# eckertzhang/Text2NeRF

Hardware: AMD Instinct MI355X
Metric: ray-samples/s (render) + iters/s (train), 300^3 VM-split, 800x800 (higher is better)
Workload: dtype f32 (basis/MLP products as f16x2-split MFMA, fp32 accumulate); 1 GPU; C2 300^3 800x800 view/GPU, N=518, S1-soft seed 0, white_bg, weights=0, tile marcher; evaluated_samples_per_frame=77423712, appearance_samples_per_frame=4284741, rays_per_gpu=640000, samples_per_ray=518, warmup_frames=231, inregion_timing=none, parallelism=ray-tile x1

## Files before the change

### include/t2n.h

```cpp
#ifndef T2N_H_
#define T2N_H_

#include <stddef.h>
#include <stdint.h>

#ifdef __cplusplus
extern "C" {
#endif

typedef struct t2n_field t2n_field;
typedef void* t2n_stream;

enum {
    T2N_OK = 0,
    T2N_ERR_INVALID = -1,
    T2N_ERR_UNSUPPORTED = -2,
    T2N_ERR_HIP = -3,
    T2N_ERR_WORKSPACE = -4,
    T2N_ERR_STATE = -5
};

enum { T2N_SHADE_MLP_FEA_NOVIEW = 0, T2N_SHADE_SH = 1, T2N_SHADE_RGB = 2,
       T2N_SHADE_MLP_FEA = 3, T2N_SHADE_MLP_PE = 4, T2N_SHADE_MLP = 5 };
enum { T2N_ACT_SOFTPLUS = 0, T2N_ACT_RELU = 1 };
// ... 37 lines not shown
    const float* app_plane[3];
    const float* app_line[3];
    const float* basis_weight;
    const float* mlp_w0; const float* mlp_b0;
    const float* mlp_w1; const float* mlp_b1;
    const float* mlp_w2; const float* mlp_b2;
} t2n_field_params;

typedef struct t2n_field_grads {
    float* density_plane[3];
    float* density_line[3];
    float* app_plane[3];
    float* app_line[3];
    float* basis_weight;
    float* mlp_w0; float* mlp_b0;
    float* mlp_w1; float* mlp_b1;
    float* mlp_w2; float* mlp_b2;
} t2n_field_grads;

enum { T2N_STAT_EVALUATED = 0,
       T2N_STAT_APPEARANCE = 1,
       T2N_STAT_RAYS = 2,
       T2N_STAT_OVERFLOW = 3,
       T2N_STAT_F16_REDO = 4,
       T2N_STAT_LIST_RETRY = 5,
       T2N_STAT_COUNT = 8 };

const char* t2n_last_error(void);
int t2n_version(void);

int t2n_field_create(const t2n_field_desc* desc, t2n_field** out);
int t2n_field_destroy(t2n_field* f);
int t2n_field_upload(t2n_field* f, const t2n_field_params* p, t2n_stream stream);
int t2n_field_set_desc(t2n_field* f, const t2n_field_desc* desc);
int t2n_field_set_factor_storage(t2n_field* f, int bf16);

int t2n_field_set_mlp_precision(t2n_field* f, int exact_fp32);
int t2n_field_set_alpha_mask(t2n_field* f, const float* volume, int D, int H, int W, const float* aabb_min_host,
                             const float* inv_size_host, t2n_stream stream);
int t2n_alpha_at(const t2n_field* f, const float* xyz_world, int64_t n, float* alpha, t2n_stream stream);
int t2n_field_set_early_termination(t2n_field* f, float eps);
int t2n_field_set_feature_staging(t2n_field* f, int on);
int t2n_field_feature_staging_counts(const t2n_field* f, uint64_t out[2]);
int t2n_field_set_density_cache(t2n_field* f, int on);
int t2n_field_set_density_cache_cap(t2n_field* f, uint64_t bytes);
int t2n_field_release_density_cache(t2n_field* f);
int t2n_field_density_cache_counts(const t2n_field* f, uint64_t out[4]);
int t2n_field_density_sum_table(const t2n_field* f, const int* shift, float* out, t2n_stream stream);
#define T2N_APP_VOLUME_MIN_FRAMES 33
int t2n_field_set_appearance_volume(t2n_field* f, int on, int min_frames);
int t2n_field_set_appearance_volume_cap(t2n_field* f, uint64_t bytes);
int t2n_field_release_appearance_volume(t2n_field* f);
int t2n_field_appearance_volume_counts(const t2n_field* f, uint64_t out[4]);
int t2n_field_feature_rows(t2n_field* f, const float* app_pos, const uint32_t* counters, uint32_t list_cap, int volume, float* feat,
                           uint32_t feat_rows, t2n_stream stream);
int t2n_field_set_feature_stage_shape(t2n_field* f, int workgroups, int defer_cap);
int t2n_field_set_frame_width(t2n_field* f, int width);

int t2n_ray_directions(int H, int W, float fx, float fy, float cx, float cy, int normalize, float* dirs ,
                       t2n_stream stream);
int t2n_get_rays(const float* dirs , int64_t n, const float* c2w_host ,
                 float* rays_o , float* rays_d , float* rays6 ,
                 t2n_stream stream);
int t2n_generate_rays(int H, int W, float fx, float fy, float cx, float cy, const float* c2w_host, float* rays6,
                      t2n_stream stream);

int t2n_sample_ray(const t2n_field* f, const float* rays_o, const float* rays_d, int64_t n, int n_samples, const float* jitter, int ndc,
                   float* pts , float* z_vals , uint8_t* valid , t2n_stream stream);

int t2n_filter_rays_bbox(const t2n_field* f, const float* rays, int64_t n_rays, int ray_stride, uint8_t* mask,
                         t2n_stream stream);

int t2n_density_at(const t2n_field* f, const float* xyz_norm, int64_t n, float* feat, float* sigma, t2n_stream stream);
size_t t2n_shade_workspace_bytes(int64_t n);
int t2n_shade_at(const t2n_field* f, const float* xyz_norm, const float* viewdirs, int64_t n, float* app_feat, float* rgb,
                 void* workspace, size_t workspace_bytes, t2n_stream stream);
int t2n_raw2alpha(const float* sigma, const float* dist, int64_t n_rays, int n_samples, float* alpha, float* weights,
                  float* bg, t2n_stream stream);

size_t t2n_render_workspace_bytes(int64_t rays_per_launch, int n_samples);
size_t t2n_render_head_scratch_bytes(const t2n_field* f, int64_t n_rays);
int t2n_field_set_head_scratch_rows(t2n_field* f, int rows_per_ray);
size_t t2n_render_workspace_bytes_hint(const t2n_field* f, int64_t n_rays, int n_samples);
size_t t2n_render_workspace_bytes_budget(int64_t n_rays, int n_samples, int entries_per_ray);
uint64_t t2n_field_list_retries(const t2n_field* f);
int t2n_render_forward(t2n_field* f, const float* rays, int64_t n_rays, int ray_stride, int n_samples, uint32_t flags,
                       const float* jitter, float* rgb, float* depth, float* weights, float* z_vals, uint64_t* stats,
                       void* workspace, size_t workspace_bytes, t2n_stream stream);

typedef struct t2n_generic_desc {
    float aabb_min[3], aabb_max[3], inv_aabb_size[3];
    int32_t grid[3];
    int32_t density_n_comp[3], app_n_comp[3];
    int32_t app_dim, shading, fea_pe, view_pe, feature_c, act;
    float density_shift, distance_scale, weight_thres, step_size, near, far, z_gate;
    const float* alpha_volume;
    int32_t alpha_dims[3];
    float alpha_aabb_min[3], alpha_aabb_max[3];
} t2n_generic_desc;
size_t t2n_generic_workspace_bytes(int64_t n_rays, int n_samples);
size_t t2n_generic_workspace_bytes_desc(const t2n_generic_desc* desc, int64_t n_rays, int n_samples);
int t2n_generic_forward(const t2n_generic_desc* desc, const t2n_field_params* params, const float* rays, int64_t n_rays, int ray_stride,
                        int n_samples, uint32_t flags, const float* jitter, float* rgb, float* depth, float* weights, float* z_vals,
                        uint64_t* stats, void* workspace, size_t workspace_bytes, t2n_stream stream);
int t2n_generic_backward(const t2n_generic_desc* desc, const t2n_field_params* params, const float* rays, int64_t n_rays, int ray_stride,
                         int n_samples, uint32_t flags, const float* jitter, const float* weights, const float* z_vals,
// ... 240 lines not shown
```

### text2nerf_amd/_lib.py

```python
from __future__ import annotations

import ctypes as C
import os
import threading

_HERE = os.path.dirname(os.path.abspath(__file__))
LIB_PATH = os.environ.get("T2N_LIB") or os.path.join(_HERE, "libt2n_hip.so")

T2N_STAT_COUNT = 8
T2N_K_COUNT = 14
KERNEL_NAMES = ("march", "shade", "composite", "upload", "bwd_march", "bwd_mlp", "bwd_scatter", "density", "app_features",
                "bwd_wgrad", "bwd_density", "tv_seed", "adam", "head_step")
STAT_EVALUATED, STAT_APPEARANCE, STAT_RAYS, STAT_OVERFLOW, STAT_F16_REDO, STAT_LIST_RETRY = 0, 1, 2, 3, 4, 5

FLAG_TRAIN, FLAG_ADD_BG, FLAG_KEEP_CTX, FLAG_COHERENT, FLAG_NDC = 1, 2, 4, 8, 16
FLAG_DEVICE_ROWS = 32
FLAG_PIPELINE = 64
FLAG_GATHER_BATCH = 128
FLAG_REG_L1, FLAG_REG_ORTHO = 256, 512
REG_SLOTS = 64
SHADE_IDS = {"MLP_Fea_noview": 0, "SH": 1, "RGB": 2, "MLP_Fea": 3, "MLP_PE": 4, "MLP": 5}
ACT_IDS = {"softplus": 0, "relu": 1}
DEPTH_KINDS = {"mse": 0, "gnll": 1, "si_log": 2, "ssi": 3}
MASK_U8, MASK_I32, MASK_I64, MASK_F32, MASK_F64 = 0, 1, 2, 3, 4
# ... 32 lines not shown
                ("alpha_aabb_max", C.c_float * 3)]


class GenericBwdPlan(C.Structure):
    _fields_ = [("kernel_form", C.c_int), ("pass_rows", C.c_uint32), ("max_passes", C.c_uint32), ("workspace_bytes", C.c_size_t)]


TRAIN_HYPER_FLOATS = 32
TRAIN_HEAD_GRAD_FLOATS = 27 * 144 + 128 * 351 + 128 + 128 * 128 + 128 + 3 * 128 + 3 + 1
TRAIN_HEAD_SIZES = (27 * 144, 128 * 351, 128, 128 * 128, 128, 3 * 128, 3)


class TrainStepArgs(C.Structure):
    _fields_ = [("rays", C.c_void_p), ("n_rays", C.c_int64), ("ray_stride", C.c_int32), ("n_samples", C.c_int32),
                ("flags", C.c_uint32), ("phases", C.c_uint32),
                ("jitter", C.c_void_p), ("rgb_target", C.c_void_p), ("depth_target", C.c_void_p),
                ("w_depth", C.c_float), ("w_trans", C.c_float), ("delta", C.c_float),
                ("beta1", C.c_float), ("beta2", C.c_float), ("eps", C.c_float),
                ("hyper", C.c_void_p), ("params", FieldParams),
                ("exp_avg", C.c_void_p * 19), ("exp_avg_sq", C.c_void_p * 19),
                ("head_grads", C.c_void_p), ("rows_capacity", C.c_int64),
                ("workspace", C.c_void_p), ("workspace_bytes", C.c_size_t), ("losses", C.c_void_p), ("host_batch", C.c_void_p), ("host_batch_bytes", C.c_size_t), ("batch_buffer", C.c_void_p),
                ("shard_world", C.c_int32), ("shard_rank", C.c_int32)]


class TrainSource(C.Structure):
    _fields_ = [("rays", C.c_void_p), ("ray_stride", C.c_int32), ("rgb", C.c_void_p), ("depth", C.c_void_p), ("n_rows", C.c_int64),
                ("ids", C.c_void_p)]


_lib = None
_lock = threading.Lock()

SIGNATURES = {
    "t2n_last_error": (C.c_char_p, []),
    "t2n_version": (C.c_int, []),
    "t2n_field_create": (C.c_int, [C.POINTER(FieldDesc), C.POINTER(C.c_void_p)]),
    "t2n_field_destroy": (C.c_int, [C.c_void_p]),
    "t2n_field_upload": (C.c_int, [C.c_void_p, C.POINTER(FieldParams), C.c_void_p]),
    "t2n_field_set_desc": (C.c_int, [C.c_void_p, C.POINTER(FieldDesc)]),
    "t2n_field_set_mlp_precision": (C.c_int, [C.c_void_p, C.c_int]),
    "t2n_field_set_early_termination": (C.c_int, [C.c_void_p, C.c_float]),
    "t2n_field_set_feature_staging": (C.c_int, [C.c_void_p, C.c_int]),
    "t2n_field_feature_staging_counts": (C.c_int, [C.c_void_p, C.POINTER(C.c_uint64)]),
    "t2n_field_set_feature_stage_shape": (C.c_int, [C.c_void_p, C.c_int, C.c_int]),
    "t2n_field_set_density_cache": (C.c_int, [C.c_void_p, C.c_int]),
    "t2n_field_set_density_cache_cap": (C.c_int, [C.c_void_p, C.c_uint64]),
    "t2n_field_release_density_cache": (C.c_int, [C.c_void_p]),
    "t2n_field_density_cache_counts": (C.c_int, [C.c_void_p, C.POINTER(C.c_uint64)]),
    "t2n_field_set_appearance_volume": (C.c_int, [C.c_void_p, C.c_int, C.c_int]),
    "t2n_field_set_appearance_volume_cap": (C.c_int, [C.c_void_p, C.c_uint64]),
    "t2n_field_release_appearance_volume": (C.c_int, [C.c_void_p]),
    "t2n_field_appearance_volume_counts": (C.c_int, [C.c_void_p, C.POINTER(C.c_uint64)]),
    "t2n_field_feature_rows": (C.c_int, [C.c_void_p, C.c_void_p, C.c_void_p, C.c_uint32, C.c_int, C.c_void_p, C.c_uint32, C.c_void_p]),
    "t2n_field_density_sum_table": (C.c_int, [C.c_void_p, C.POINTER(C.c_int), C.c_void_p, C.c_void_p]),
    "t2n_sample_ray": (C.c_int, [C.c_void_p, C.c_void_p, C.c_void_p, C.c_int64, C.c_int, C.c_void_p, C.c_int, C.c_void_p, C.c_void_p,
                                 C.c_void_p, C.c_void_p]),
    "t2n_field_set_frame_width": (C.c_int, [C.c_void_p, C.c_int]),
    "t2n_field_set_alpha_mask": (C.c_int, [C.c_void_p, C.c_void_p, C.c_int, C.c_int, C.c_int, C.POINTER(C.c_float),
                                           C.POINTER(C.c_float), C.c_void_p]),
    "t2n_alpha_at": (C.c_int, [C.c_void_p, C.c_void_p, C.c_int64, C.c_void_p, C.c_void_p]),
    "t2n_ray_directions": (C.c_int, [C.c_int, C.c_int, C.c_float, C.c_float, C.c_float, C.c_float, C.c_int,
                                     C.c_void_p, C.c_void_p]),
    "t2n_get_rays": (C.c_int, [C.c_void_p, C.c_int64, C.POINTER(C.c_float), C.c_void_p, C.c_void_p, C.c_void_p,
                               C.c_void_p]),
    "t2n_generate_rays": (C.c_int, [C.c_int, C.c_int, C.c_float, C.c_float, C.c_float, C.c_float,
                                    C.POINTER(C.c_float), C.c_void_p, C.c_void_p]),
    "t2n_filter_rays_bbox": (C.c_int, [C.c_void_p, C.c_void_p, C.c_int64, C.c_int, C.c_void_p, C.c_void_p]),
    "t2n_density_at": (C.c_int, [C.c_void_p, C.c_void_p, C.c_int64, C.c_void_p, C.c_void_p, C.c_void_p]),
    "t2n_shade_workspace_bytes": (C.c_size_t, [C.c_int64]),
    "t2n_shade_at": (C.c_int, [C.c_void_p, C.c_void_p, C.c_void_p, C.c_int64, C.c_void_p, C.c_void_p, C.c_void_p,
                               C.c_size_t, C.c_void_p]),
    "t2n_raw2alpha": (C.c_int, [C.c_void_p, C.c_void_p, C.c_int64, C.c_int, C.c_void_p, C.c_void_p, C.c_void_p,
                                C.c_void_p]),
    "t2n_render_workspace_bytes": (C.c_size_t, [C.c_int64, C.c_int]),
    "t2n_render_head_scratch_bytes": (C.c_size_t, [C.c_void_p, C.c_int64]),
    "t2n_field_set_head_scratch_rows": (C.c_int, [C.c_void_p, C.c_int]),
    "t2n_render_workspace_bytes_hint": (C.c_size_t, [C.c_void_p, C.c_int64, C.c_int]),
    "t2n_field_list_retries": (C.c_uint64, [C.c_void_p]),
    "t2n_render_workspace_bytes_budget": (C.c_size_t, [C.c_int64, C.c_int, C.c_int]),
    "t2n_render_forward": (C.c_int, [C.c_void_p, C.c_void_p, C.c_int64, C.c_int, C.c_int, C.c_uint32, C.c_void_p,
                                     C.c_void_p, C.c_void_p, C.c_void_p, C.c_void_p, C.c_void_p, C.c_void_p,
                                     C.c_size_t, C.c_void_p]),
    "t2n_render_workspace_bytes_ctx": (C.c_size_t, [C.c_int64, C.c_int]),
    "t2n_depth_align_global": (C.c_int, [C.c_void_p, C.c_void_p, C.c_int, C.c_int, C.c_void_p, C.c_int, C.c_double, C.c_void_p, C.c_void_p,
                                         C.c_void_p]),
    "t2n_depth_align_fallback": (C.c_int, [C.c_void_p, C.c_void_p, C.c_int, C.c_int, C.c_double, C.c_void_p, C.c_void_p, C.c_void_p]),
    "t2n_filled_pixels_workspace_bytes": (C.c_size_t, [C.c_int, C.c_int]),
    "t2n_filled_pixels_count": (C.c_int, [C.c_void_p, C.c_int, C.c_int, C.c_void_p, C.c_void_p, C.c_void_p]),
    "t2n_filled_pixels_select": (C.c_int, [C.c_void_p, C.c_int, C.c_int, C.c_void_p, C.c_void_p, C.c_int, C.c_void_p, C.c_void_p]),
    "t2n_depth_merge_inputs": (C.c_int, [C.c_void_p, C.c_void_p, C.c_void_p, C.c_int, C.c_int, C.c_double, C.c_void_p, C.c_void_p,
                                         C.c_void_p, C.c_void_p]),
    "t2n_view_finish": (C.c_int, [C.c_void_p, C.c_void_p, C.c_void_p, C.c_int, C.c_int, C.c_double, C.c_void_p, C.c_void_p, C.c_void_p,
                                  C.c_void_p]),
    "t2n_mask_expand": (C.c_int, [C.c_void_p, C.c_int, C.c_int, C.c_void_p, C.c_void_p, C.c_void_p]),
    "t2n_mc_workspace_bytes": (C.c_size_t, [C.c_int, C.c_int, C.c_int]),
    "t2n_mc_count": (C.c_int, [C.c_void_p, C.c_int, C.c_int, C.c_int, C.c_float, C.c_void_p, C.c_void_p, C.c_void_p]),
    "t2n_mc_emit": (C.c_int, [C.c_void_p, C.c_int, C.c_int, C.c_int, C.c_float, C.c_void_p, C.POINTER(C.c_float), C.POINTER(C.c_float),
                              C.c_int, C.c_void_p, C.c_void_p, C.c_void_p, C.c_void_p]),
    "t2n_mesh_components_workspace_bytes": (C.c_size_t, [C.c_int64, C.c_int64]),
    "t2n_mesh_components": (C.c_int, [C.c_void_p, C.c_int64, C.c_int64, C.c_void_p, C.c_void_p, C.c_void_p, C.c_size_t, C.c_void_p]),
    "t2n_mesh_component_sizes": (C.c_int, [C.c_void_p, C.c_int64, C.c_void_p, C.c_int64, C.c_int64, C.c_void_p, C.c_void_p, C.c_void_p]),
    "t2n_mesh_filter_count": (C.c_int, [C.c_void_p, C.c_int64, C.c_void_p, C.c_int64, C.c_void_p, C.c_int64, C.c_void_p, C.c_size_t,
                                        C.c_void_p, C.c_void_p]),
    "t2n_mesh_filter_emit": (C.c_int, [C.c_void_p, C.c_int64, C.c_void_p, C.c_int64, C.c_void_p, C.c_int64, C.c_void_p, C.c_void_p,
                                       C.c_void_p, C.c_void_p, C.c_size_t, C.c_void_p, C.c_void_p, C.c_void_p, C.c_void_p, C.c_void_p]),
# ... 159 lines not shown
```

### text2nerf_amd/build.py

```python
from __future__ import annotations

import concurrent.futures
import glob
import os
import subprocess
import sys

HERE = os.path.dirname(os.path.abspath(__file__))
ROOT = os.path.dirname(HERE)
CSRC = os.path.join(HERE, "csrc")
LIB = os.path.join(HERE, "libt2n_hip.so")
OBJ = os.path.join(ROOT, "build", "obj")

CFLAGS = ["--offload-arch=gfx950", "-O3", "-std=c++17", "-fPIC", "-ffp-contract=off", "-fno-fast-math",
          "-munsafe-fp-atomics", "-Wall", "-Wno-unused-function", "-DNDEBUG"]
LDFLAGS = ["--offload-arch=gfx950", "-shared", "-fPIC",
           "-Wl,--no-undefined"]
FLAGS = CFLAGS + LDFLAGS[1:]
PER_FILE = {"t2n_mlp_bwd_ss.hip": ["-fno-slp-vectorize"]}


def sources():
    return sorted(glob.glob(os.path.join(CSRC, "*.hip")))


def _headers():
    return glob.glob(os.path.join(CSRC, "*.h")) + [os.path.join(ROOT, "include", "t2n.h"), __file__]


def _obj(src):
    return os.path.join(OBJ, os.path.basename(src)[:-4] + ".o")


def _stale(src):
    o = _obj(src)
    if not os.path.exists(o):
        return True
    t = os.path.getmtime(o)
    return os.path.getmtime(src) > t or any(os.path.getmtime(h) > t for h in _headers())


def needs_build():
    if not os.path.exists(LIB):
        return True
    t = os.path.getmtime(LIB)
    return any(os.path.getmtime(d) > t for d in sources() + _headers())


def check_ss3_isa(hipcc, verbose=False, extra=(), obj_dir=None):
    import re
    obj_dir = obj_dir or OBJ
    src = os.path.join(CSRC, "t2n_mlp_ss.hip")
    asm = os.path.join(obj_dir, "t2n_mlp_ss.s")
    subprocess.run([hipcc] + CFLAGS + list(extra) + ["-S", "--cuda-device-only", src, "-o", asm], check=True,
                   stderr=subprocess.DEVNULL)
    text = open(asm).read()
    found = 0
    for m in re.finditer(r"^(_ZN3t2n2ss9k_mlp_ss3\w*):[^\n]*\n(.*?)\n\.Lfunc_end\d+:", text, re.S | re.M):
        name, body = m.group(1), m.group(2)
        found += 1
        bad = [l.strip() for l in body.split("\n") if re.match(r"\s*v_accvgpr_(write|mov)", l)]
        meta = re.search(r"\.name:\s+" + name + r"\n.*?\.vgpr_spill_count:\s+(\d+)", text, re.S)
        priv = re.search(r"\.name:\s+" + name + r"\n.*?\.private_segment_fixed_size:\s+(\d+)", text, re.S)
        spills = int(meta.group(1)) if meta else -1
        scratch = int(priv.group(1)) if priv else -1
        if bad or spills != 0 or scratch != 0:
            raise RuntimeError(f"{name}: the compiler touched the AccVGPRs or spilled ({len(bad)} v_accvgpr_write/mov, {spills} spilled "
                               f"registers, {scratch} B of scratch): the hand-allocated accumulators are not safe with this build")
        if verbose:
            print(f"check_ss3_isa: {name} ok ({body.count('v_accvgpr_read_b32')} accumulator reads, no writes, no spills)", flush=True)
    if found != 2:
        raise RuntimeError(f"check_ss3_isa: expected the two instantiations of k_mlp_ss3 in the assembly, found {found}")


def build(force=False, verbose=False):
    if not force and not needs_build():
        return LIB
    hipcc = os.environ.get("HIPCC", "/opt/rocm/bin/hipcc")
    os.makedirs(OBJ, exist_ok=True)
    todo = [s for s in sources() if force or _stale(s)]

    def compile_one(src):
        cmd = [hipcc] + CFLAGS + PER_FILE.get(os.path.basename(src), []) + ["-c", src, "-o", _obj(src)]
        if verbose:
            print(" ".join(cmd), flush=True)
        subprocess.run(cmd, check=True)

    with concurrent.futures.ThreadPoolExecutor(max_workers=min(8, max(1, len(todo)))) as ex:
        list(ex.map(compile_one, todo))
    ss_obj = _obj(os.path.join(CSRC, "t2n_mlp_ss.hip"))
    stamp = ss_obj[:-2] + ".checked"
    if not os.path.exists(stamp) or os.path.getmtime(stamp) < os.path.getmtime(ss_obj):
        try:
            check_ss3_isa(hipcc, verbose)
        except Exception:
            for f in (ss_obj, stamp):
                if os.path.exists(f):
                    os.remove(f)
            raise
        open(stamp, "w").close()
    keep = {_obj(s) for s in sources()}
    for o in glob.glob(os.path.join(OBJ, "*.o")):
        if o not in keep:
            os.remove(o)
    cmd = [hipcc] + LDFLAGS + sorted(keep) + ["-o", LIB + ".tmp"]
    if verbose:
        print(" ".join(cmd), flush=True)
    subprocess.run(cmd, check=True)
    os.replace(LIB + ".tmp", LIB)
    return LIB


if __name__ == "__main__":
    if "--check-ss3" in sys.argv:
        i = sys.argv.index("--check-ss3")
        check_ss3_isa(os.environ.get("HIPCC", "/opt/rocm/bin/hipcc"), True, extra=sys.argv[i + 2:], obj_dir=sys.argv[i + 1])
        sys.exit(0)
    print(build(force="--force" in sys.argv, verbose=True))
```

### text2nerf_amd/csrc/t2n_api.hip

```cpp
#include <stdarg.h>

#include "t2n_device.h"

namespace t2n {

static thread_local char g_err[512] = "";

void set_error(const char* fmt, ...) {
    va_list ap;
    va_start(ap, fmt);
    vsnprintf(g_err, sizeof(g_err), fmt, ap);
    va_end(ap);
}

int hip_fail(hipError_t e, const char* what) {
    set_error("HIP error %d (%s) in %s", (int)e, hipGetErrorString(e), what);
    return T2N_ERR_HIP;
}

void timing_begin(t2n_field* f, int k, hipStream_t s) {
    if (!((f->timing >> k) & 1)) return;
    TimingSlot& t = f->slots[k];
    if (t.used >= kTimingEvents) return;
    if (!t.start[t.used]) {
// ... 277 lines not shown
    if (deg < 3) return;
    o[9] = (-0.5900435899266435f * y) * (3.f * xx - yy);
    o[10] = (2.890611442640554f * xy) * z;
    o[11] = (-0.4570457994644658f * y) * ((4.f * zz - xx) - yy);
    o[12] = (0.3731763325901154f * z) * ((2.f * zz - 3.f * xx) - 3.f * yy);
    o[13] = (-0.4570457994644658f * x) * ((4.f * zz - xx) - yy);
    o[14] = (1.445305721320277f * z) * (xx - yy);
    o[15] = (-0.5900435899266435f * x) * (xx - 3.f * yy);
    if (deg < 4) return;
    o[16] = (2.5033429417967046f * xy) * (xx - yy);
    o[17] = (-1.7701307697799304f * yz) * (3.f * xx - yy);
    o[18] = (0.9461746957575601f * xy) * (7.f * zz - 1.f);
    o[19] = (-0.6690465435572892f * yz) * (7.f * zz - 3.f);
    o[20] = 0.10578554691520431f * (zz * (35.f * zz - 30.f) + 3.f);
    o[21] = (-0.6690465435572892f * xz) * (7.f * zz - 3.f);
    o[22] = (0.47308734787878004f * (xx - yy)) * (7.f * zz - 1.f);
    o[23] = (-1.7701307697799304f * xz) * (xx - 3.f * yy);
    o[24] = 0.6258357354491761f * (xx * (xx - 3.f * yy) - yy * (3.f * xx - yy));
}

__global__ __launch_bounds__(256) void k_ndc_rays(int H, int W, float focal, float near, float sign, const float* __restrict__ ro,
                                                  const float* __restrict__ rd, long long n, float* o_out, float* d_out) {
    const long long i = (long long)blockIdx.x * blockDim.x + threadIdx.x;
    if (i >= n) return;
    float ox = ro[i * 3], oy = ro[i * 3 + 1], oz = ro[i * 3 + 2];
    const float dx = rd[i * 3], dy = rd[i * 3 + 1], dz = rd[i * 3 + 2];
    const float t = sign < 0.f ? -(near + oz) / dz : (near - oz) / dz;
    ox = ox + t * dx; oy = oy + t * dy; oz = oz + t * dz;
    const float kx = sign * 1.f / ((float)W / (2.f * focal)), ky = sign * 1.f / ((float)H / (2.f * focal));
    const float o0 = kx * ox / oz, o1 = ky * oy / oz;
    const float o2 = sign < 0.f ? 1.f + 2.f * near / oz : 1.f - 2.f * near / oz;
    const float d0 = kx * (dx / dz - ox / oz), d1 = ky * (dy / dz - oy / oz);
    const float d2 = sign < 0.f ? -2.f * near / oz : 2.f * near / oz;
    o_out[i * 3] = o0; o_out[i * 3 + 1] = o1; o_out[i * 3 + 2] = o2;
    d_out[i * 3] = d0; d_out[i * 3 + 1] = d1; d_out[i * 3 + 2] = d2;
}

static size_t align_up(size_t x, size_t a) { return (x + a - 1) / a * a; }

Carve carve_workspace(int64_t rays, int n_samples, bool ctx, bool feat, unsigned budget) {
    Carve c;
    c.list_cap = list_capacity_budget(rays, n_samples, budget);
    const size_t cap = (size_t)c.list_cap * kLists;
    size_t o = 0;
    c.counters = o; o = align_up(o + (size_t)kLists * kCounterStride * 4, 256);
    c.acc = o; o = align_up(o + (size_t)rays * 4, 256);
    c.ray_app = o; o = align_up(o + (size_t)rays * 16, 256);
    c.app_pos = o; o = align_up(o + cap * 16, 256);
    c.app_rgb = o; o = align_up(o + cap * 16, 256);
    c.app_ray = o; o = align_up(o + cap * 4, 256);
    c.sigma = o; if (ctx) o = align_up(o + (size_t)rays * n_samples * 4, 256);
    c.rgb_raw = o; if (ctx) o = align_up(o + (size_t)rays * 16, 256);
    c.scratch = o; if (ctx) o = align_up(o + (size_t)rays * (size_t)(n_samples / 4 > 0 ? n_samples / 4 : 1) * 16 + 256 + (size_t)rays * 4, 256);
    const size_t worst_rows = cap + (size_t)kLists * 32, want_rows = (size_t)rays * (budget && budget < 64 ? (budget + 1) / 2 : 32) + 1024;
    c.feat_rows = (unsigned)(((worst_rows < want_rows ? worst_rows : want_rows) + 127) / 128 * 128);
    if (!feat) c.feat_rows = 0;
    c.feat = o; o = align_up(o + (size_t)c.feat_rows * 32 * sizeof(float), 256);
    c.total = o;
    return c;
}
static Carve carve(int64_t rays, int n_samples) { return carve_workspace(rays, n_samples, true); }
constexpr unsigned kBudgetMin = 16;
constexpr unsigned kBudgetFloor = 2;
constexpr int64_t kBudgetMinRays = 65536;

}

using namespace t2n;

extern "C" const char* t2n_last_error(void) { return g_err; }
extern "C" int t2n_version(void) { return 100; }

extern "C" int t2n_field_create(const t2n_field_desc* desc, t2n_field** out) {
    if (!desc || !out) { set_error("t2n_field_create: NULL argument"); return T2N_ERR_INVALID; }
    t2n_field* f = new t2n_field();
    memset(&f->dev, 0, sizeof(f->dev));
    for (int k = 0; k < T2N_K_COUNT; ++k) { memset(f->slots[k].start, 0, sizeof(f->slots[k].start)); memset(f->slots[k].stop, 0, sizeof(f->slots[k].stop)); }
    const int rc = apply_desc(f, desc);
    if (rc) { delete f; return rc; }
    *out = f;
    return T2N_OK;
}

extern "C" int t2n_field_set_desc(t2n_field* f, const t2n_field_desc* d) {
    if (!f || !d) { set_error("t2n_field_set_desc: NULL argument"); return T2N_ERR_INVALID; }
    if (f->uploaded && (d->grid[0] != f->desc.grid[0] || d->grid[1] != f->desc.grid[1] || d->grid[2] != f->desc.grid[2] ||
                        d->density_n_comp != f->desc.density_n_comp || d->app_n_comp != f->desc.app_n_comp)) {
        set_error("t2n_field_set_desc: grid/n_comp change needs a new field handle");
        return T2N_ERR_STATE;
    }
    return apply_desc(f, d);
}

extern "C" int t2n_field_destroy(t2n_field* f) {
    if (!f) return T2N_OK;
    for (int k = 0; k < 3; ++k) {
        if (f->buf_den_plane[k]) (void)hipFree(f->buf_den_plane[k]);
        if (f->buf_den_line[k]) (void)hipFree(f->buf_den_line[k]);
        if (f->buf_app_plane[k]) (void)hipFree(f->buf_app_plane[k]);
        if (f->buf_app_line[k]) (void)hipFree(f->buf_app_line[k]);
        if (f->hbuf_den_plane[k]) (void)hipFree(f->hbuf_den_plane[k]);
        if (f->hbuf_den_line[k]) (void)hipFree(f->hbuf_den_line[k]);
        if (f->hbuf_app_plane[k]) (void)hipFree(f->hbuf_app_plane[k]);
        if (f->hbuf_app_line[k]) (void)hipFree(f->hbuf_app_line[k]);
    }
    if (f->gbuf_all && !f->gbuf_external) (void)hipFree(f->gbuf_all);
    if (f->buf_mlp) (void)hipFree(f->buf_mlp);
// ... 267 lines not shown
        if (carve_workspace(n_rays, n_samples, true, false).total > workspace_bytes || (uint64_t)list_capacity(n_rays, n_samples) * kLists > 0x7fffffffull) {
            set_error("t2n_render_forward: KEEP_CTX needs the whole call in one launch (workspace %zu B < %zu B)", workspace_bytes,
                      carve_workspace(n_rays, n_samples, true, false).total);
            return T2N_ERR_WORKSPACE;
        }
        if (!weights || !z_vals) { set_error("t2n_render_forward: KEEP_CTX needs weights and z_vals materialised"); return T2N_ERR_INVALID; }
    }
    int64_t per = n_rays;
    unsigned budget = 0;
    counts_poll(f, false);
    const bool generic_head = head_is_generic(f->desc.shading);
    if (tiles && !generic_head && carve(n_rays, n_samples).total > workspace_bytes && n_rays >= kBudgetMinRays && !getenv("T2N_NO_BUDGET")) {
        unsigned lo = 0, hi = (unsigned)n_samples;
        if (carve_workspace(n_rays, n_samples, true, true, kBudgetFloor).total <= workspace_bytes) {
            lo = kBudgetFloor;
            while (hi - lo > 1) {
                const unsigned mid = lo + (hi - lo) / 2;
                if (carve_workspace(n_rays, n_samples, true, true, mid).total <= workspace_bytes) lo = mid; else hi = mid;
            }
        }
        if (lo >= kBudgetFloor && (uint64_t)list_capacity_budget(n_rays, n_samples, lo) * kLists <= 0x7fffffffull) budget = lo;
    }

    const size_t head_row_bytes = generic_head ? (size_t)(32 + head_dims(f->desc).K0pad + 128 + 128) * sizeof(float) : 0;
    auto head_bytes = [&](int64_t rays) { return generic_head ? ((size_t)rays * (size_t)f->head_rows_per_ray + 32 * kLists) / 32 * 32 * head_row_bytes + 256 : (size_t)0; };
    if (!budget) {
        while (!keep && per > 1 && carve(per, n_samples).total + head_bytes(per) > workspace_bytes) per = (per + 1) / 2;
        if (!keep && carve(per, n_samples).total + head_bytes(per) > workspace_bytes) { set_error("t2n_render_forward: workspace %zu B too small", workspace_bytes); return T2N_ERR_WORKSPACE; }
        while ((uint64_t)list_capacity(per, n_samples) * kLists > 0x7fffffffull) per = (per + 1) / 2;
        if (tiles && per < n_rays) {
            const int64_t band = (int64_t)8 * f->frame_w;
            per = per / band * band;
            if (per <= 0) { set_error("t2n_render_forward: workspace too small for one 8-row band"); return T2N_ERR_WORKSPACE; }
        }
    }
    if (tiles) { const int rc = density_cache_prepare(f, s); if (rc) return rc; }
    AvolScope avol_scope{f};
    if (tiles) { const int rc = appearance_volume_prepare(f, s); if (rc) return rc; }
    char* ws = (char*)workspace;
    for (int64_t off = 0; off < n_rays; off += per) {
        const int64_t cnt = (n_rays - off) < per ? (n_rays - off) : per;
        const Carve c = carve_workspace(per, n_samples, true, !keep, budget);
        RenderLaunch L;
        L.rays = rays + off * ray_stride; L.n_rays = cnt; L.ray_stride = ray_stride; L.n_samples = n_samples; L.flags = flags;
        L.jitter = (jitter && !ndc) ? jitter + off : jitter;
        L.rgb = rgb + off * 3; L.depth = depth + off;
        L.weights = weights ? weights + off * n_samples : nullptr;
        L.z_vals = z_vals ? z_vals + off * n_samples : nullptr;
        L.stats = stats;
        L.counters = (unsigned*)(ws + c.counters); L.acc = (float*)(ws + c.acc); L.ray_app = (int4*)(ws + c.ray_app);
        L.app_pos = (float4*)(ws + c.app_pos); L.app_rgb = (float4*)(ws + c.app_rgb); L.app_ray = (int*)(ws + c.app_ray);
        L.list_cap = c.list_cap;
        L.feat = (float*)(ws + c.feat); L.feat_rows = c.feat_rows;
        L.sigma_ctx = keep ? (float*)(ws + c.sigma) : nullptr;
        L.rgb_raw = keep ? (float4*)(ws + c.rgb_raw) : nullptr;
        int rc;
        const KeptRows kr = keep && f->desc.shading == T2N_SHADE_MLP_FEA_NOVIEW ? kept_rows(c.total, workspace_bytes) : KeptRows{0, 0, 0, 0, 0};
        {
            SetupOps so;
            const bool mark = kr.rows >= 32;
            if (!mark) so.zero(L.counters, (size_t)kLists * kCounterStride * 4);
            else {
                const unsigned lo = kKeptMagicWord < kKeptRowsWord ? kKeptMagicWord : kKeptRowsWord, hi = kKeptMagicWord < kKeptRowsWord ? kKeptRowsWord : kKeptMagicWord;
                so.zero(L.counters, (size_t)lo * 4);
                if (hi > lo + 1) so.zero(L.counters + lo + 1, (size_t)(hi - lo - 1) * 4);
                if ((unsigned)(kLists * kCounterStride) > hi + 1) so.zero(L.counters + hi + 1, (size_t)(kLists * kCounterStride - hi - 1) * 4);
                so.set(L.counters + kKeptMagicWord, kKeptMagic);
                so.set(L.counters + kKeptRowsWord, (unsigned)kr.rows);
            }
            if (stats_pending) { so.zero(stats, sizeof(uint64_t) * T2N_STAT_COUNT); stats_pending = false; }
            if (tiles) {
                const int cap_e = n_samples / 4 > 0 ? n_samples / 4 : 1;
                so.zero(ws + c.scratch + (size_t)cnt * cap_e * 16, 4);
            }
            if ((rc = launch_setup(so, s))) return rc;
        }
        if (tiles) {
            if ((rc = launch_march_tiles(f, L, f->frame_w, (int)(cnt / f->frame_w), (float*)(ws + c.sigma), (float4*)(ws + c.scratch), s))) return rc;
        } else if ((rc = launch_march(f, L, s))) return rc;
        if (budget) counts_post(f, L.counters, n_rays, n_samples, budget, s);
        if (keep && (rc = ctx_counts_post(workspace, L.counters, s))) return rc;
        if (generic_head) {
            const HeadDims H = head_dims(f->desc);
            HeadPlanDev* plan = (HeadPlanDev*)(L.counters + kHeadPlanWord);
            if ((rc = launch_head_plan(L.counters, L.list_cap, plan, s))) return rc;
            const size_t off = align_up(c.total, 256);
            size_t avail = workspace_bytes > off ? workspace_bytes - off : 0;
            long long cap = (long long)(avail / head_row_bytes) / 32 * 32;
            if (cap > 0x7fffffe0ll) cap = 0x7fffffe0ll;
            if (cap < 32) {
                set_error("t2n_render_forward: the workspace holds no activation row of the general head (add t2n_render_head_scratch_bytes)");
                return T2N_ERR_WORKSPACE;
            }
            {
                float* feat32 = (float*)(ws + off); float* x0 = feat32 + cap * 32; float* h0 = x0 + cap * H.K0pad; float* h1 = h0 + cap * 128;
                const long long worst = ((long long)L.list_cap + 31) / 32 * 32 * kLists;
                const long long worst_rows = worst < (cnt * (long long)n_samples + 32ll * kLists) ? worst : (cnt * (long long)n_samples + 32ll * kLists);
                for (long long row0 = 0; row0 < worst_rows; row0 += cap) {
                    ShadeCtx ctx{nullptr, feat32 - row0 * 32, nullptr, nullptr};
                    if ((rc = launch_shade_list(f, L.app_pos, L.app_ray, L.rays, ray_stride, L.counters, L.list_cap, L.app_rgb, &ctx, s, true,
                                                (unsigned)(row0 + cap), nullptr, 0, nullptr, (unsigned)(row0 / 32), (unsigned)((row0 + cap) / 32)))) return rc;
                    if ((rc = launch_head_forward(f, nullptr, cap, feat32, L.app_pos, L.app_ray, L.rays, ray_stride, L.counters, L.list_cap, x0, h0,
                                                  h1, L.app_rgb, s, plan, row0))) return rc;
                }
            }
        } else {
            if (kr.rows >= 32) {
                ShadeCtx ctx{(float*)(ws + kr.x144), (float*)(ws + kr.feat32), (float*)(ws + kr.h0), (float*)(ws + kr.h1)};
                if ((rc = launch_shade_list(f, L.app_pos, L.app_ray, L.rays, ray_stride, L.counters, L.list_cap, L.app_rgb, &ctx, s, false, kr.rows))) return rc;
            } else if ((rc = launch_shade_list(f, L.app_pos, L.app_ray, L.rays, ray_stride, L.counters, L.list_cap, L.app_rgb, nullptr, s, false,
                                               0xffffffffu, keep ? nullptr : L.feat, L.feat_rows, stats))) return rc;
        }
        if ((rc = tiles ? launch_composite(f, L, s, f->frame_w, (int)(cnt / f->frame_w)) : launch_composite(f, L, s))) return rc;
        if (tiles && finish_supported(f) && (rc = launch_finish_rays(f, L, (const float*)(ws + c.sigma), (const float4*)(ws + c.scratch), s))) return rc;
    }
    return T2N_OK;
}

extern "C" size_t t2n_render_workspace_bytes_hint(const t2n_field* f, int64_t n_rays, int n_samples) {
    if (!f || n_rays <= 0 || n_samples <= 0) return 0;
    counts_poll(const_cast<t2n_field*>(f), false);
    const size_t worst = carve(n_rays, n_samples).total;
    if (n_rays < kBudgetMinRays) return worst;
    unsigned b = f->list_hint ? 2u * f->list_hint + 16u : 32u;
    if (b < kBudgetMin) b = kBudgetMin;
    if (b >= (unsigned)n_samples) return worst;
    const size_t want = carve_workspace(n_rays, n_samples, true, true, b).total;
    return want < worst ? want : worst;
}
extern "C" uint64_t t2n_field_list_retries(const t2n_field* f) {
    if (!f) return 0;
    counts_poll(const_cast<t2n_field*>(f), true);
    return f->list_retries;
}
extern "C" size_t t2n_render_workspace_bytes_budget(int64_t n_rays, int n_samples, int entries_per_ray) {
    if (n_rays <= 0 || n_samples <= 0 || entries_per_ray < 0) return 0;
    return carve_workspace(n_rays, n_samples, true, true, (unsigned)entries_per_ray).total;
}

extern "C" int t2n_field_set_alpha_mask(t2n_field* f, const float* volume, int D, int H, int W, const float* aabb_min_host,
                                        const float* inv_size_host, t2n_stream stream) {
    if (!f) { set_error("t2n_field_set_alpha_mask: NULL field"); return T2N_ERR_INVALID; }
    if (f->buf_alpha) { T2N_HIP(hipStreamSynchronize((hipStream_t)stream)); (void)hipFree(f->buf_alpha); f->buf_alpha = nullptr; }
    f->dev.alpha = nullptr;
    if (!volume) return T2N_OK;
    if (D < 1 || H < 1 || W < 1 || !aabb_min_host || !inv_size_host) { set_error("t2n_field_set_alpha_mask: bad argument"); return T2N_ERR_INVALID; }
    const size_t bytes = (size_t)D * H * W * sizeof(float);
    T2N_HIP(hipMalloc((void**)&f->buf_alpha, bytes));
    T2N_HIP(hipMemcpyAsync(f->buf_alpha, volume, bytes, hipMemcpyDeviceToDevice, (hipStream_t)stream));
    f->dev.alpha = f->buf_alpha; f->dev.aD = D; f->dev.aH = H; f->dev.aW = W;
    for (int k = 0; k < 3; ++k) { f->dev.a_min[k] = aabb_min_host[k]; f->dev.a_inv[k] = inv_size_host[k]; }
    return T2N_OK;
}

extern "C" int t2n_field_set_head_scratch_rows(t2n_field* f, int rows_per_ray) {
    if (!f || rows_per_ray < 1 || rows_per_ray > 4096) { set_error("t2n_field_set_head_scratch_rows: rows_per_ray must lie in [1, 4096]"); return T2N_ERR_INVALID; }
    f->head_rows_per_ray = rows_per_ray;
    return T2N_OK;
}

extern "C" int t2n_field_set_frame_width(t2n_field* f, int width) {
    if (!f || width < 0) { set_error("t2n_field_set_frame_width: bad argument"); return T2N_ERR_INVALID; }
    f->frame_w = width;
    return T2N_OK;
}

extern "C" int t2n_field_set_factor_storage(t2n_field* f, int bf16) {
    if (!f) { set_error("t2n_field_set_factor_storage: NULL field"); return T2N_ERR_INVALID; }
    if ((bf16 != 0) != (f->factor_bf16 != 0)) f->uploaded = false;
    f->factor_bf16 = bf16 ? 1 : 0;
    if (!f->factor_bf16)
        for (int k = 0; k < 3; ++k) {
            f->dev.den.plane_h[k] = f->dev.den.line_h[k] = f->dev.app.plane_h[k] = f->dev.app.line_h[k] = nullptr;
        }
    return T2N_OK;
}

// ... 9 lines not shown
extern "C" int t2n_field_set_mlp_precision(t2n_field* f, int exact_fp32) {
    if (!f) { set_error("t2n_field_set_mlp_precision: NULL field"); return T2N_ERR_INVALID; }
    f->mlp_split = exact_fp32 ? 0 : 1;
    return T2N_OK;
}

extern "C" int t2n_field_set_feature_staging(t2n_field* f, int on) {
    if (!f) { set_error("t2n_field_set_feature_staging: NULL field"); return T2N_ERR_INVALID; }
    f->feature_staging = on ? 1 : 0;
    return T2N_OK;
}

extern "C" int t2n_field_set_density_cache(t2n_field* f, int on) {
    if (!f) { set_error("t2n_field_set_density_cache: NULL field"); return T2N_ERR_INVALID; }
    f->dcache_on = on ? 1 : 0;
    return T2N_OK;
}
extern "C" int t2n_field_set_density_cache_cap(t2n_field* f, uint64_t bytes) {
    if (!f) { set_error("t2n_field_set_density_cache_cap: NULL field"); return T2N_ERR_INVALID; }
    f->dcache_cap = (size_t)bytes;
    f->dcache_alloc_failed = false;
    return T2N_OK;
}
extern "C" int t2n_field_release_density_cache(t2n_field* f) {
    if (!f) { set_error("t2n_field_release_density_cache: NULL field"); return T2N_ERR_INVALID; }
    density_cache_release(f);
    return T2N_OK;
}
extern "C" int t2n_field_density_cache_counts(const t2n_field* f, uint64_t out[4]) {
    if (!f || !out) { set_error("t2n_field_density_cache_counts: NULL argument"); return T2N_ERR_INVALID; }
    out[0] = f->dcache_counts[0]; out[1] = f->dcache_counts[1]; out[2] = f->dcache_counts[2]; out[3] = (uint64_t)f->dcache_bytes;
    return T2N_OK;
}
extern "C" int t2n_field_set_appearance_volume(t2n_field* f, int on, int min_frames) {
    if (!f || min_frames < 0) { set_error("t2n_field_set_appearance_volume: NULL field or min_frames < 0"); return T2N_ERR_INVALID; }
    f->avol_on = on ? 1 : 0;
    f->avol_min_frames = min_frames ? min_frames : T2N_APP_VOLUME_MIN_FRAMES;
    return T2N_OK;
}
extern "C" int t2n_field_set_appearance_volume_cap(t2n_field* f, uint64_t bytes) {
    if (!f) { set_error("t2n_field_set_appearance_volume_cap: NULL field"); return T2N_ERR_INVALID; }
    f->avol_cap = (size_t)bytes;
    f->avol_alloc_failed = false;
    return T2N_OK;
}
extern "C" int t2n_field_release_appearance_volume(t2n_field* f) {
    if (!f) { set_error("t2n_field_release_appearance_volume: NULL field"); return T2N_ERR_INVALID; }
    appearance_volume_release(f);
    return T2N_OK;
}
extern "C" int t2n_field_appearance_volume_counts(const t2n_field* f, uint64_t out[4]) {
    if (!f || !out) { set_error("t2n_field_appearance_volume_counts: NULL argument"); return T2N_ERR_INVALID; }
    out[0] = (uint64_t)f->avol_bytes; out[1] = f->avol_counts[2]; out[2] = f->avol_counts[0]; out[3] = f->avol_counts[1];
    return T2N_OK;
}
extern "C" int t2n_field_feature_rows(t2n_field* f, const float* app_pos, const uint32_t* counters, uint32_t list_cap, int volume, float* feat,
                                      uint32_t feat_rows, t2n_stream stream) {
    if (!f || !app_pos || !counters || !feat || feat_rows % 32u) { set_error("t2n_field_feature_rows: bad argument"); return T2N_ERR_INVALID; }
    if (!f->uploaded) { set_error("t2n_field_feature_rows: the field has no uploaded parameters"); return T2N_ERR_STATE; }
    if (f->desc.shading != T2N_SHADE_MLP_FEA_NOVIEW || !f->mlp_split) { set_error("t2n_field_feature_rows: needs the fused MLP_Fea_noview head on split products"); return T2N_ERR_UNSUPPORTED; }
    hipStream_t s = (hipStream_t)stream;
    AvolScope avol_scope{f};
    f->dev.avol = nullptr;
    if (volume) {
        const int on = f->avol_on, mf = f->avol_min_frames;
        f->avol_on = 1; f->avol_min_frames = 1;
        const int rc = appearance_volume_prepare(f, s);
        f->avol_on = on; f->avol_min_frames = mf;
        if (rc) return rc;
        if (!f->dev.avol) { set_error("t2n_field_feature_rows: this field gets no feature volume (cap, addressing, allocation)"); return T2N_ERR_UNSUPPORTED; }
    }
    return launch_feature_rows(f, (const float4*)app_pos, counters, list_cap, feat, feat_rows, s);
}
extern "C" int t2n_field_density_sum_table(const t2n_field* f, const int* shift, float* out, t2n_stream stream) {
    if (!f || !shift || !out) { set_error("t2n_field_density_sum_table: NULL argument"); return T2N_ERR_INVALID; }
    if (!f->uploaded) { set_error("t2n_field_density_sum_table: the field has no uploaded factors"); return T2N_ERR_STATE; }
    return launch_density_sum_table(f, out, shift, (hipStream_t)stream);
}

extern "C" int t2n_field_set_feature_stage_shape(t2n_field* f, int workgroups, int defer_cap) {
    if (!f) { set_error("t2n_field_set_feature_stage_shape: NULL field"); return T2N_ERR_INVALID; }
    if (workgroups < 0 || defer_cap < 0 || defer_cap > 64) { set_error("t2n_field_set_feature_stage_shape: workgroups >= 0, defer_cap in [0, 64]"); return T2N_ERR_INVALID; }
    f->feature_workgroups = workgroups;
    f->feature_defer_cap = defer_cap ? defer_cap : 16;
    return T2N_OK;
}

extern "C" int t2n_field_feature_staging_counts(const t2n_field* f, uint64_t out[2]) {
    if (!f || !out) { set_error("t2n_field_feature_staging_counts: NULL argument"); return T2N_ERR_INVALID; }
    out[0] = out[1] = 0;
    if (!f->staging_counts) return T2N_OK;
    T2N_HIP(hipDeviceSynchronize());
    unsigned long long h[2];
    T2N_HIP(hipMemcpy(h, f->staging_counts, sizeof(h), hipMemcpyDeviceToHost));
    out[0] = h[0]; out[1] = h[1];
    return T2N_OK;
}

extern "C" int t2n_timing_enable(t2n_field* f, int on) {
    if (!f) return T2N_ERR_INVALID;
    f->timing = on == 0 ? 0 : (on == 1 ? (1 << T2N_K_COUNT) - 1 : (on >> 1) & ((1 << T2N_K_COUNT) - 1));
    return T2N_OK;
}

extern "C" int t2n_timing_read(t2n_field* f, double* ms, int64_t* launches, int reset) {
    if (!f || !ms || !launches) { set_error("t2n_timing_read: NULL argument"); return T2N_ERR_INVALID; }
// ... 8 lines not shown
```

### text2nerf_amd/csrc/t2n_app_volume.hip

```cpp
#include "t2n_internal.h"
#include "t2n_device.h"

namespace t2n {

constexpr int kAvK = 144;

struct AvBuildArgs { FactorSet app; const float* Bt; float* out; int n[3]; long long corners; };

template <int K>
__device__ __forceinline__ void av_pair(const AvBuildArgs& a, const float* __restrict__ Bs, const int c[3], float (&acc)[28]) {
    const float4* __restrict__ P = reinterpret_cast<const float4*>(a.app.plane[K]) + ((size_t)c[mat1(K)] * a.app.W[K] + c[mat0(K)]) * 12;
    const float4* __restrict__ L = reinterpret_cast<const float4*>(a.app.line[K]) + (size_t)c[vecm(K)] * 12;
#pragma unroll 1
    for (int q = 0; q < 12; ++q) {
        const float4 p = P[q], l = L[q];
        const float x[4] = {p.x * l.x, p.y * l.y, p.z * l.z, p.w * l.w};
        const float4* __restrict__ b = reinterpret_cast<const float4*>(Bs + (48 * K + 4 * q) * 32);
#pragma unroll
        for (int ch = 0; ch < 4; ++ch)
#pragma unroll
            for (int jq = 0; jq < 7; ++jq) {
                const float4 bv = b[ch * 8 + jq];
                acc[4 * jq] = fmaf(bv.x, x[ch], acc[4 * jq]); acc[4 * jq + 1] = fmaf(bv.y, x[ch], acc[4 * jq + 1]);
                acc[4 * jq + 2] = fmaf(bv.z, x[ch], acc[4 * jq + 2]); acc[4 * jq + 3] = fmaf(bv.w, x[ch], acc[4 * jq + 3]);
            }
    }
}

__global__ __launch_bounds__(256) void k_app_volume_build(const AvBuildArgs a) {
    __shared__ __attribute__((aligned(16))) float Bs[kAvK * 32];
    for (int i = threadIdx.x; i < kAvK * 32 / 4; i += 256) reinterpret_cast<float4*>(Bs)[i] = reinterpret_cast<const float4*>(a.Bt)[i];
    __syncthreads();
    const long long idx = (long long)blockIdx.x * 256 + threadIdx.x;
    if (idx >= a.corners) return;
    const int nx = a.n[0] + 1, ny = a.n[1] + 1;
    const int x = (int)(idx % nx), y = (int)((idx / nx) % ny), z = (int)(idx / ((long long)nx * ny));
    const int c[3] = {min(x, a.n[0] - 1), min(y, a.n[1] - 1), min(z, a.n[2] - 1)};
    float acc[28];
#pragma unroll
    for (int j = 0; j < 28; ++j) acc[j] = 0.f;
    av_pair<0>(a, Bs, c, acc);
    av_pair<1>(a, Bs, c, acc);
    av_pair<2>(a, Bs, c, acc);
    float4* __restrict__ o = reinterpret_cast<float4*>(a.out + (size_t)idx * kAvStride);
#pragma unroll
    for (int jq = 0; jq < 7; ++jq) o[jq] = make_float4(acc[4 * jq], acc[4 * jq + 1], acc[4 * jq + 2], jq == 6 ? 0.f : acc[4 * jq + 3]);
    if constexpr (kAvStride == 32) o[7] = make_float4(0.f, 0.f, 0.f, 0.f);
}

struct AvReadArgs {
    FactorSet app;
    const float* avol; unsigned row, slice, ny1;
    const float4* app_pos; const unsigned* counters; unsigned list_cap; int nlists; unsigned tile_hi;
    float* feat;
};

__global__ __launch_bounds__(256) void k_app_features_vol(const AvReadArgs a) {
    constexpr int LPE = 4, NQ = 8 / LPE, EPP = 64 / LPE, PASSES = 32 / EPP;
    const int lane = threadIdx.x & 63, wid = __builtin_amdgcn_readfirstlane((int)(threadIdx.x >> 6));
    unsigned cnt_l = 0;
    if (lane < a.nlists) {
        cnt_l = a.counters[lane * kCounterStride];
        if (cnt_l > a.list_cap) cnt_l = a.list_cap;
    }
    unsigned incl = (cnt_l + 31u) / 32u;
#pragma unroll
    for (int o = 1; o < 8; o <<= 1) {
        const unsigned t = __shfl_up(incl, o);
        if (lane >= o) incl += t;
    }
    unsigned ntiles = (unsigned)__builtin_amdgcn_readfirstlane((int)__shfl(incl, a.nlists - 1));
    if (ntiles > a.tile_hi) ntiles = a.tile_hi;
    const unsigned wave_stride = gridDim.x * 4u;
    const int e = lane / LPE, q = lane % LPE;
    const char* __restrict__ V = reinterpret_cast<const char*>(a.avol);
    for (unsigned tile = blockIdx.x * 4u + wid; tile < ntiles; tile += wave_stride) {
        const int li = (int)__popcll(__ballot((lane < a.nlists) & (incl <= tile)));
        const unsigned before = li ? __shfl(incl, li - 1) : 0u;
        const unsigned lbase = (unsigned)li * a.list_cap;
        const unsigned base = (unsigned)__builtin_amdgcn_readfirstlane((int)(lbase + (tile - before) * 32u));
        const unsigned count = lbase + __shfl(cnt_l, li);
        const unsigned nlive = (unsigned)__builtin_amdgcn_readfirstlane((int)(count - base < 32u ? count - base : 32u));
        const float4* __restrict__ pb = a.app_pos + base;
        asm volatile("" : "+s"(pb));
        float* __restrict__ rb = a.feat + (size_t)tile * 1024;
        asm volatile("" : "+s"(rb));
        float4 pos[PASSES];
#pragma unroll
        for (int p = 0; p < PASSES; ++p) pos[p] = (unsigned)(EPP * p + e) < nlive ? pb[EPP * p + e] : make_float4(0.f, 0.f, 0.f, 0.f);
#pragma unroll
        for (int p = 0; p < PASSES; ++p) {
            const bool live = (unsigned)(EPP * p + e) < nlive;
            const float4 mine = pos[p];
            const Axes3 A = sample_axes_inbox(a.app, mine.x, mine.y, mine.z);
            const unsigned ix = (unsigned)min(max(A.a[0].i0, 0), a.app.W[0] - 1), iy = (unsigned)min(max(A.a[1].i0, 0), a.app.H[0] - 1);
            const unsigned iz = (unsigned)min(max(A.a[2].i0, 0), a.app.H[1] - 1);
            const unsigned cell = umad24(umad24(iz, a.ny1, iy), a.row, ix * kAvCornerBytes);
            const unsigned o00 = (live ? cell : 0u) + (unsigned)q * 16u;
            const unsigned o01 = o00 + a.row, o10 = o00 + a.slice, o11 = o10 + a.row;
            const unsigned off[4] = {o00, o01, o10, o11};
            float4 c[4][2][NQ];
#pragma unroll
            for (int zy = 0; zy < 4; ++zy)
#pragma unroll
                for (int x = 0; x < 2; ++x)
#pragma unroll
                    for (int i = 0; i < NQ; ++i)
                        c[zy][x][i] = *reinterpret_cast<const float4*>(V + (size_t)off[zy] + ((int)kAvCornerBytes * x + 16 * LPE * i));
            __builtin_amdgcn_sched_barrier(0);
            const float wx0 = live ? A.a[0].w0 : 0.f, wx1 = live ? A.a[0].w1 : 0.f;
            const float wyx[2][2] = {{A.a[1].w0 * wx0, A.a[1].w0 * wx1}, {A.a[1].w1 * wx0, A.a[1].w1 * wx1}};
            const float wz[2] = {A.a[2].w0, A.a[2].w1};
            float4 r[NQ];
#pragma unroll
            for (int zy = 0; zy < 4; ++zy)
#pragma unroll
                for (int x = 0; x < 2; ++x) {
                    const float w = wyx[zy & 1][x] * wz[zy >> 1];
#pragma unroll
                    for (int i = 0; i < NQ; ++i) r[i] = (zy == 0 && x == 0) ? f4_mul(c[0][0][i], w) : f4_fma(c[zy][x][i], w, r[i]);
                }
            if (q == 6 % LPE) r[6 / LPE].w = live ? mine.w : 0.f;
            if (q == 7 % LPE) r[7 / LPE] = make_float4(0.f, 0.f, 0.f, 0.f);
            float* __restrict__ row = rb + (unsigned)((EPP * p + e) * 32 + 4 * q);
#pragma unroll
            for (int i = 0; i < NQ; ++i) *reinterpret_cast<float4*>(row + 4 * LPE * i) = r[i];
        }
    }
}

int launch_app_features_vol(t2n_field* f, const float4* app_pos, const unsigned* counters_dev, unsigned list_cap, unsigned tile_hi, float* feat,
                            hipStream_t s) {
    AvReadArgs a;
    a.app = f->dev.app;
    a.avol = f->dev.avol; a.row = f->dev.av_row; a.slice = f->dev.av_slice; a.ny1 = (unsigned)f->desc.grid[1] + 1u;
    a.app_pos = app_pos; a.counters = counters_dev; a.list_cap = list_cap; a.nlists = kLists; a.tile_hi = tile_hi; a.feat = feat;
    const unsigned long long wg = ((unsigned long long)tile_hi + 3u) / 4u;
    const unsigned wg_max = 256u * 8u;
    const dim3 grid((unsigned)(wg < wg_max ? (wg ? wg : 1u) : wg_max));
    hipLaunchKernelGGL(k_app_features_vol, grid, dim3(256), 0, s, a);
    T2N_HIP(hipGetLastError());
    return T2N_OK;
}

size_t appearance_volume_bytes(const t2n_field* f) {
    const int* g = f->desc.grid;
    return (size_t)(g[0] + 1) * (g[1] + 1) * (g[2] + 1) * kAvCornerBytes;
}

int launch_app_volume_build(const t2n_field* f, float* out, hipStream_t s) {
    AvBuildArgs a;
    a.app = f->dev.app; a.Bt = f->dev.basisA; a.out = out;
    a.corners = 1;
    for (int k = 0; k < 3; ++k) { a.n[k] = f->desc.grid[k]; a.corners *= a.n[k] + 1; }
    hipLaunchKernelGGL(k_app_volume_build, dim3((unsigned)((a.corners + 255) / 256)), dim3(256), 0, s, a);
    T2N_HIP(hipGetLastError());
    return T2N_OK;
}

void appearance_volume_release(t2n_field* f) {
    if (f->avol) { (void)hipDeviceSynchronize(); (void)hipFree(f->avol); }
    f->avol = nullptr; f->avol_bytes = 0; f->avol_version = 0; f->avol_seen = 0; f->avol_run = 0; f->avol_alloc_failed = false;
    f->dev.avol = nullptr;
}

int appearance_volume_prepare(t2n_field* f, hipStream_t s) {
    f->dev.avol = nullptr;
    if (f->avol_seen == f->app_version) ++f->avol_run; else { f->avol_seen = f->app_version; f->avol_run = 1; }
    const auto direct = [&]() { ++f->avol_counts[1]; return (int)T2N_OK; };
    if (!f->avol_on) return direct();
    if (f->desc.shading != T2N_SHADE_MLP_FEA_NOVIEW || !f->mlp_split || f->desc.app_n_comp != 48 || f->desc.app_dim != 27) return direct();
    const int* g = f->desc.grid;
    const size_t bytes = appearance_volume_bytes(f);
    size_t cap = f->avol_cap;
    if (!cap) {
        static size_t dev_total[64] = {};
        int d = 0;
        if (hipGetDevice(&d) != hipSuccess) { (void)hipGetLastError(); d = 0; }
        size_t& total = dev_total[(unsigned)d % 64u];
// ... 36 lines not shown
```

### text2nerf_amd/csrc/t2n_internal.h

```cpp
#pragma once
#include <hip/hip_runtime.h>
#include <stdint.h>
#include <stdio.h>
#include <string.h>

#include "../../include/t2n.h"

namespace t2n {

constexpr int kWave = 64;
constexpr int kMaxSamples = 8192;
constexpr int kAppDimMax = 32;

__host__ __device__ constexpr int mat0(int k) { return k == 2 ? 1 : 0; }
__host__ __device__ constexpr int mat1(int k) { return k == 0 ? 1 : 2; }
__host__ __device__ constexpr int vecm(int k) { return 2 - k; }

struct FactorSet {
    const float* plane[3];
    const float* line[3];
    int W[3], H[3], L[3];
    int C;
    const void* plane_h[3];
    const void* line_h[3];
// ... 57 lines not shown
    void* buf_mlp_h = nullptr;
    const unsigned* split_unsafe = nullptr;
    void* buf_ss = nullptr;
    bool ss_dirty = true;
    void* ss_event = nullptr; void* ss_stream = nullptr;
    unsigned* ss_ok_host = nullptr; void* ss_ok_event = nullptr; int ss_variant = -2;
    float* buf_alpha = nullptr;
    int mlp_split = 1;
    int feature_staging = 1;
    unsigned long long* staging_counts = nullptr;
    int feature_defer_cap = 16;
    int feature_workgroups = 0;
    float* gbuf_den_plane[3] = {nullptr, nullptr, nullptr};
    float* gbuf_den_line[3] = {nullptr, nullptr, nullptr};
    float* gbuf_app_plane[3] = {nullptr, nullptr, nullptr};
    float* gbuf_app_line[3] = {nullptr, nullptr, nullptr};
    bool gbuf_external = false;
    float* gbuf_all = nullptr; size_t gbuf_bytes = 0;
    t2n_field_params params_ref;
    bool uploaded = false;
    int timing = 0;
    int frame_w = 0;
    int head_rows_per_ray = 32;
    float term_eps = 0.f;
    t2n::TimingSlot slots[T2N_K_COUNT];
    static constexpr int kCountSlots = 4;
    struct CountSlot { unsigned* host = nullptr; void* ev = nullptr; bool pending = false; int64_t n_rays = 0; int n_samples = 0; unsigned budget = 0; };
    CountSlot count_slots[kCountSlots]; int count_next = 0;
    void* side_stream = nullptr; void* ev_fork = nullptr; void* ev_join = nullptr;
    void* ev_den = nullptr;
    unsigned* plan_host = nullptr; unsigned plan_seq = 0;
    void* ev_pack = nullptr;
    void* gemm_stream = nullptr; void* ev_fork2 = nullptr; void* ev_join2 = nullptr;
    void* train_dev = nullptr; unsigned* train_host = nullptr; void* train_ev[12] = {};
    unsigned train_calls = 0; bool train_chain = false;
    bool train_packed = false;
    t2n_train_source train_src = {}; bool train_src_set = false;
    bool train_src_fresh = false;
    unsigned list_hint = 0;
    void* reg_ws = nullptr; size_t reg_ws_bytes = 0;
    unsigned long long list_retries = 0;
    float* dcache = nullptr; size_t dcache_bytes = 0;
    unsigned long long den_version = 1, dcache_version = 0, dcache_seen = 0;
    int dcache_on = 1; size_t dcache_cap = 0;
    bool dcache_alloc_failed = false;
    void* dcache_ev = nullptr; void* dcache_stream = nullptr;
    unsigned long long dcache_counts[3] = {0, 0, 0};
    float* avol = nullptr; size_t avol_bytes = 0;
    unsigned long long app_version = 1, avol_version = 0, avol_seen = 0, avol_run = 0;
    int avol_on = 1, avol_min_frames = T2N_APP_VOLUME_MIN_FRAMES; size_t avol_cap = 0;
    bool avol_alloc_failed = false;
    void* avol_ev = nullptr; void* avol_stream = nullptr;
    unsigned long long avol_counts[3] = {0, 0, 0};
};

namespace t2n {

void set_error(const char* fmt, ...);
int hip_fail(hipError_t e, const char* what);

#define T2N_HIP(call)                                        \
    do {                                                     \
        hipError_t e__ = (call);                             \
        if (e__ != hipSuccess) return t2n::hip_fail(e__, #call); \
    } while (0)

void counts_poll(t2n_field* f, bool wait);
void timing_begin(t2n_field* f, int k, hipStream_t s);
void timing_end(t2n_field* f, int k, hipStream_t s);

int launch_relayout(t2n_field* f, const t2n_field_params* p, hipStream_t s);
int launch_pack_mlp(t2n_field* f, const t2n_field_params* p, hipStream_t s, unsigned* absmax_out = nullptr);

struct RenderLaunch {
    const float* rays; int64_t n_rays; int ray_stride; int n_samples; uint32_t flags;
    const float* jitter; float* rgb; float* depth; float* weights; float* z_vals; uint64_t* stats;
    float* acc; int4* ray_app; unsigned* counters; float4* app_pos; int* app_ray; float4* app_rgb; unsigned list_cap;
    float* feat = nullptr; unsigned feat_rows = 0;
    float* sigma_ctx; float4* rgb_raw;
};
int launch_march(t2n_field* f, const RenderLaunch& L, hipStream_t s);
int launch_ray_stats(const RenderLaunch& L, hipStream_t s);
int launch_filter_bbox(const FieldDev& F, const float* rays, long long n_rays, int ray_stride, uint8_t* mask, hipStream_t s);
int launch_filter_alpha(const FieldDev& F, const float* rays, long long n_rays, int ray_stride, int n_samples, uint8_t* mask, hipStream_t s);
size_t density_cache_bytes(const t2n_field* f);
int density_cache_prepare(t2n_field* f, hipStream_t s);
void density_cache_release(t2n_field* f);
int launch_density_sum_table(const t2n_field* f, float* out, const int shift[3], hipStream_t s);
#ifndef T2N_AVOL_STRIDE
#define T2N_AVOL_STRIDE 32
#endif
constexpr int kAvStride = T2N_AVOL_STRIDE;
constexpr int kAvFeatures = 27;
constexpr unsigned kAvCornerBytes = kAvStride * sizeof(float);
static_assert(kAvStride % 4 == 0 && kAvStride >= 28 && kAvStride <= 32, "corner stride: whole quads that hold the 27 features");
struct AvolScope { t2n_field* f; ~AvolScope() { f->dev.avol = nullptr; } };
size_t appearance_volume_bytes(const t2n_field* f);
int appearance_volume_prepare(t2n_field* f, hipStream_t s);
void appearance_volume_release(t2n_field* f);
int launch_app_volume_build(const t2n_field* f, float* out, hipStream_t s);
int launch_app_features_vol(t2n_field* f, const float4* app_pos, const unsigned* counters_dev, unsigned list_cap, unsigned tile_hi, float* feat,
                            hipStream_t s);
int launch_feature_rows(t2n_field* f, const float4* app_pos, const unsigned* counters_dev, unsigned list_cap, float* feat, unsigned feat_rows,
                        hipStream_t s);
int launch_march_tiles(t2n_field* f, const RenderLaunch& L, int img_w, int img_h, float* spill, float4* scratch, hipStream_t s);
constexpr int kLists = 8;
constexpr int kCounterStride = 64;
inline unsigned list_capacity(long long n_rays, int n_samples) {
    const unsigned nblocks = (unsigned)((n_rays + 3) / 4);
    return ((nblocks >> 3) + ((nblocks & 7u) ? 1u : 0u)) * 4u * (unsigned)n_samples + (unsigned)n_samples;
}
inline unsigned list_capacity_budget(long long n_rays, int n_samples, unsigned budget) {
    const unsigned worst = list_capacity(n_rays, n_samples);
    if (budget == 0 || budget >= (unsigned)n_samples) return worst;
    const unsigned long long per = ((unsigned long long)n_rays * budget + kLists - 1) / kLists + (unsigned)n_samples;
    return per < worst ? (unsigned)per : worst;
}
struct ShadeCtx { float* x144; float* feat32; float* h0; float* h1; };
int launch_shade_list(t2n_field* f, const float4* app_pos, const int* app_ray, const float* rays, int ray_stride,
                      const unsigned* counters_dev, unsigned list_cap, float4* app_rgb, const ShadeCtx* ctx, hipStream_t s,
                      bool features_only = false, unsigned ctx_rows = 0xffffffffu, float* feat = nullptr, unsigned feat_rows = 0,
                      uint64_t* stats = nullptr, unsigned tile_lo = 0, unsigned tile_hi = 0xffffffffu);
constexpr int kRangeFlagWord = 32;
constexpr int kKeptMagicWord = 33, kKeptRowsWord = 34;
constexpr int kOverflowWord = 35;
constexpr int kHeadPlanWord = 40;
constexpr int kFailEntriesWord = 36;
constexpr unsigned kKeptMagic = 0x4b455054u;
int launch_mlp_ss(t2n_field* f, const float* feat, const unsigned* counters_dev, unsigned list_cap, unsigned tile_hi, float4* app_rgb,
                  unsigned* range_flag, hipStream_t s);

struct HeadDims { int shading, C, fea_pe, view_pe, pos_pe, o_feat, o_view, o_pe_a, n_pe_a, o_pe_v, n_pe_v, K0, K0pad; };
HeadDims head_dims(const t2n_field_desc& d);
inline bool head_is_generic(int shading) { return shading == T2N_SHADE_MLP_FEA || shading == T2N_SHADE_MLP_PE || shading == T2N_SHADE_MLP; }
struct HeadPlanDev { unsigned t[kLists + 1]; unsigned rows; };
int launch_head_plan(const unsigned* counters, unsigned list_cap, HeadPlanDev* plan, hipStream_t s);
int launch_dense_rows(const float* IN, int ldin, const float* Wt, int K, int N, const float* bias, int relu, long long rows, float* OUT, int ldo,
                      hipStream_t s, const HeadPlanDev* plan, long long row0);
int launch_head_forward(t2n_field* f, const unsigned tiles_before[kLists + 1], long long rows, const float* feat32, const float4* app_pos,
                        const int* app_ray, const float* rays, int ray_stride, const unsigned* counters, unsigned list_cap, float* x0,
                        float* h0, float* h1, float4* app_rgb, hipStream_t s, const HeadPlanDev* plan = nullptr, long long row0 = 0);
int launch_head_in_bwd(t2n_field* f, const float* gx, const float* feat32, long long rows, float* gf, hipStream_t s);
struct SetupOps {
    unsigned* zero_ptr[6]; unsigned long long zero_words[6]; int nz = 0;
    unsigned* set_ptr[4]; unsigned set_val[4]; int ns = 0;
    bool overflow = false;
    void zero(void* p, size_t bytes) {
        if (!p || !bytes) return;
        if (nz >= 6) { overflow = true; return; }
        zero_ptr[nz] = (unsigned*)p; zero_words[nz] = (bytes + 3) / 4; ++nz;
    }
    void set(void* p, unsigned v) {
        if (ns >= 4) { overflow = true; return; }
        set_ptr[ns] = (unsigned*)p; set_val[ns] = v; ++ns;
    }
};
int launch_setup(const SetupOps& o, hipStream_t s);
int launch_simple_head_bwd(t2n_field* f, const unsigned tiles_before[kLists + 1], long long rows, const float4* go, const float4* app_rgb,
                           const int* app_ray, const float* rays, int ray_stride, const unsigned* counters, unsigned list_cap, float* gf,
                           hipStream_t s);

size_t gemm_h_pack_bytes(int K0);
int gemm_h_pack(t2n_field* f, void* buf, int K0, hipStream_t s);
int launch_gemm_nn_h(void* packbuf, int which, int K0, const float* IN, int ldin, long long rows, const float* ACT, int ldact, float* OUT,
                     int ldo, hipStream_t s);
int launch_gemm_tn_b(const float* A, int lda, const float* B, int ldb, long long rows, int N, float* part, int ldp, int chunk_rows,
                     int ng, int chunks, bool pe, float* db, hipStream_t s, const unsigned* rows_dev = nullptr);
struct TnPlan { int chunk_rows, chunks, ng, ldp; };
TnPlan tn_plan(int64_t rows, int N);
size_t tn_part_bytes(int64_t rows, int k0);
bool gemm_fp32_mode(const t2n_field* f);
void launch_bwd_l2(const float4* go, const float* h1, long long rows, const float* w2, float* g1, float* dw2, float* db2, float* scratch,
                   hipStream_t s, const unsigned* rows_dev = nullptr);
void launch_gemm_tn(int MB, bool fp32, const float* A, int lda, const float* B, int ldb, long long rows, int M, int N, float* C, int ldc,
                    float* part, hipStream_t s, const float* pe_feat = nullptr, float* db = nullptr, const unsigned* rows_dev = nullptr,
                    bool reduce = true);
struct WgradRegions { size_t l2, tn[3], total; };
WgradRegions wgrad_regions(int64_t rows, int k0);
void launch_wgrad_reduce(const char* base, long long rows, float* dw2, float* db2, float* dw1, float* dw0, float* dwb, hipStream_t s,
                         const float* loss_part = nullptr, long long n_rays = 0, float w_depth = 0.f, float w_trans = 0.f, float* losses = nullptr);
void launch_gemm_nn(const float* IN, int ldin, const float* W, int ldw, long long rows, int K, int N, const float* ACT, int ldact, float* OUT,
                    int ldo, hipStream_t s);
void launch_colsum(const float* G, int ld, long long rows, int N, float* db, hipStream_t s);
// ... 41 lines not shown
```

### text2nerf_amd/csrc/t2n_march_tiles.hip

```cpp
#include "t2n_device.h"

namespace t2n {

constexpr int kMaxLog2W = 2;
constexpr int kDStrideMax = (1 << (2 * kMaxLog2W)) + 4;
constexpr int kPairFloats = 3 * 16 * kDStrideMax;
constexpr int kSumFloats = 96;
constexpr int kStageFloats = kPairFloats + kSumFloats;
static_assert(63 + 21 < kSumFloats && kStageFloats % 4 == 0, "summed table: the farthest read stays in the wave's region; 16-B aligned regions");
typedef float f32x4_t __attribute__((ext_vector_type(4)));

struct TileArgs {
    FieldDev F;
    const float* rays; long long n_rays; int ray_stride; int n_samples; int img_w, img_h;
    float* acc; float* depth; int4* ray_app;
    float* wbuf;
    float4* scratch; int cap; unsigned* ovf_count; int* ovf_list;
    float4* app_pos; int* app_ray; unsigned* counters; unsigned list_cap; unsigned long long* stats;
    float* dense_w;
#ifdef MT_PROF
    unsigned long long* prof;
#endif
};

__device__ __forceinline__ void lds_fence_w() {
    __builtin_amdgcn_fence(__ATOMIC_RELEASE, "wavefront");
    __builtin_amdgcn_wave_barrier();
    __builtin_amdgcn_fence(__ATOMIC_ACQUIRE, "wavefront");
}

template <int CTRL>
__device__ __forceinline__ int dpp_shr(int v, int identity) {
    return __builtin_amdgcn_update_dpp(identity, v, CTRL, 0xf, 0xf, false);
}
__device__ __forceinline__ int wave_min_i(int v) {
    const int big = 0x7fffffff;
    v = min(v, dpp_shr<0x111>(v, big));
    v = min(v, dpp_shr<0x112>(v, big));
    v = min(v, dpp_shr<0x114>(v, big));
    v = min(v, dpp_shr<0x118>(v, big));
    const int a = __builtin_amdgcn_readlane(v, 15), b = __builtin_amdgcn_readlane(v, 31);
    const int c = __builtin_amdgcn_readlane(v, 47), d = __builtin_amdgcn_readlane(v, 63);
    return min(min(a, b), min(c, d));
}
__device__ __forceinline__ int wave_max_i(int v) {
    const int small = -0x7fffffff;
    v = max(v, dpp_shr<0x111>(v, small));
    v = max(v, dpp_shr<0x112>(v, small));
    v = max(v, dpp_shr<0x114>(v, small));
    v = max(v, dpp_shr<0x118>(v, small));
    const int a = __builtin_amdgcn_readlane(v, 15), b = __builtin_amdgcn_readlane(v, 31);
    const int c = __builtin_amdgcn_readlane(v, 47), d = __builtin_amdgcn_readlane(v, 63);
    return max(max(a, b), max(c, d));
}

__device__ __forceinline__ unsigned wave_or_u(unsigned v) {
    v |= (unsigned)dpp_shr<0x111>((int)v, 0);
    v |= (unsigned)dpp_shr<0x112>((int)v, 0);
    v |= (unsigned)dpp_shr<0x114>((int)v, 0);
    v |= (unsigned)dpp_shr<0x118>((int)v, 0);
    const unsigned a = (unsigned)__builtin_amdgcn_readlane((int)v, 15), b = (unsigned)__builtin_amdgcn_readlane((int)v, 31);
    const unsigned c = (unsigned)__builtin_amdgcn_readlane((int)v, 47), d = (unsigned)__builtin_amdgcn_readlane((int)v, 63);
    return (a | b) | (c | d);
}

template <int LOG2W>
__device__ __forceinline__ void table_build(const FactorSet& S, const int (&amn)[3], float* __restrict__ stD, int l15, int lq) {
    constexpr int WS = 1 << LOG2W, SL = WS * WS, NB = SL / 16, ST = SL + 4;
    const int gs[3] = {S.W[0], S.H[0], S.H[1]};
    float4 av[3][NB], bv[3];
#pragma unroll
    for (int k = 0; k < 3; ++k) {
// ... 55 lines not shown
__device__ __forceinline__ CellTaps cached_load(const FieldDev& F, unsigned off) {
    const char* __restrict__ B = reinterpret_cast<const char*>(F.dsum);
    CellTaps t;
    t.d00 = *reinterpret_cast<const F2U*>(B + off);
    t.d01 = *reinterpret_cast<const F2U*>(B + (off + F.ds_row));
    t.d10 = *reinterpret_cast<const F2U*>(B + (off + F.ds_slice));
    t.d11 = *reinterpret_cast<const F2U*>(B + (off + F.ds_slice + F.ds_row));
    return t;
}
__device__ __forceinline__ float cached_read3(const Axes3& A, const CellTaps& t) {
    const Axis& ax = A.a[0];
    const Axis& ay = A.a[1];
    const Axis& az = A.a[2];
    const float wnw = ay.w0 * ax.w0, wne = ay.w0 * ax.w1, wsw = ay.w1 * ax.w0, wse = ay.w1 * ax.w1;
    float v0 = t.d00.a * wnw, v1 = t.d10.a * wnw;
    v0 = fmaf(t.d00.b, wne, v0); v1 = fmaf(t.d10.b, wne, v1);
    v0 = fmaf(t.d01.a, wsw, v0); v1 = fmaf(t.d11.a, wsw, v1);
    v0 = fmaf(t.d01.b, wse, v0); v1 = fmaf(t.d11.b, wse, v1);
    return fmaf(v1, az.w1, v0 * az.w0);
}

template <int K>
__device__ __forceinline__ float pair_dot_global(const FactorSet& S, const Axes3& A, float part) {
    const Axis& ax = A.a[mat0(K)];
    const Axis& ay = A.a[mat1(K)];
    const Axis& al = A.a[vecm(K)];
    const float4* __restrict__ P = reinterpret_cast<const float4*>(S.plane[K]);
    const float4* __restrict__ L = reinterpret_cast<const float4*>(S.line[K]);
    const unsigned W = (unsigned)S.W[K];
    const unsigned nw = ((unsigned)ay.i0 * W + ax.i0) * 4, ne = ((unsigned)ay.i0 * W + ax.i1) * 4;
    const unsigned sw = ((unsigned)ay.i1 * W + ax.i0) * 4, se = ((unsigned)ay.i1 * W + ax.i1) * 4;
#pragma unroll 1
    for (int q = 0; q < 4; ++q) {
        float4 v = f4_mul(P[nw + q], ay.w0 * ax.w0);
        v = f4_fma(P[ne + q], ay.w0 * ax.w1, v);
        v = f4_fma(P[sw + q], ay.w1 * ax.w0, v);
        v = f4_fma(P[se + q], ay.w1 * ax.w1, v);
        float4 l = f4_mul(L[al.i0 * 4 + q], al.w0);
        l = f4_fma(L[al.i1 * 4 + q], al.w1, l);
        part = fmaf(v.x, l.x, part); part = fmaf(v.y, l.y, part); part = fmaf(v.z, l.z, part); part = fmaf(v.w, l.w, part);
    }
    return part;
}

__device__ __forceinline__ void void_entries(float4* __restrict__ app_pos, int* __restrict__ app_ray, unsigned list, unsigned list_cap,
                                             unsigned lo, unsigned hi, int lane) {
    if (hi > list_cap) hi = list_cap;
    for (unsigned e = lo + (unsigned)lane; e < hi; e += 64u) {
        app_pos[(size_t)list * list_cap + e] = make_float4(0.f, 0.f, 0.f, 0.f);
        app_ray[(size_t)list * list_cap + e] = 0;
    }
}

constexpr int kDenseLd = 20;
constexpr int kDenseFloats = 64 * kDenseLd;
struct __attribute__((aligned(4))) F4U { float x, y, z, w; };

#ifndef T2N_MT_WAVES
#define T2N_MT_WAVES 5
#endif
#ifndef T2N_MTD_WAVES
#define T2N_MTD_WAVES 4
#endif
#ifndef T2N_MTC_WAVES
#define T2N_MTC_WAVES 5
#endif
#ifndef T2N_MTCD_WAVES
#define T2N_MTCD_WAVES 4
#endif
#ifdef MT_PROF
#define MT_T(var) do { const unsigned long long tn = __builtin_readcyclecounter(); var += tn - p_t; p_t = tn; } while (0)
#else
#define MT_T(var) do {} while (0)
#endif
constexpr int mt_waves(bool dense, bool cached) { return cached ? (dense ? T2N_MTCD_WAVES : T2N_MTC_WAVES) : (dense ? T2N_MTD_WAVES : T2N_MT_WAVES); }
template <bool DENSE, bool ALPHA = false, bool RELU = false, bool CACHED = false>
__global__ __launch_bounds__(256) __attribute__((amdgpu_waves_per_eu(mt_waves(DENSE, CACHED), mt_waves(DENSE, CACHED)))) void k_march_tiles(const TileArgs a) {
    extern __shared__ __attribute__((aligned(16))) float smem[];
    const int lane = threadIdx.x & 63, wid = threadIdx.x >> 6;
    const int l15 = lane & 15, lq = lane >> 4;
    float* __restrict__ stD = smem + (size_t)wid * kStageFloats;
    if constexpr (!CACHED) {
        for (int i = lane; i < kStageFloats; i += 64) stD[i] = 0.f;
        lds_fence_w();
    }
    float* __restrict__ wt = smem + (CACHED ? 0 : 4 * kStageFloats) + (size_t)wid * kDenseFloats;
    const FieldDev& F = a.F;
    const int tiles_x = (a.img_w + 7) >> 3;
    const long long tile = (long long)blockIdx.x * 4 + wid;
    const int ty = (int)(tile / tiles_x), tx = (int)(tile - (long long)ty * tiles_x);
    const int px = tx * 8 + (lane & 7), py = ty * 8 + (lane >> 3);
    if (ty * 8 >= a.img_h) return;
    const bool have = px < a.img_w && py < a.img_h;
    const long long r = have ? (long long)py * a.img_w + px : 0;
    const int N = a.n_samples;
    Ray ray;
    if (have) ray = load_ray(F, a.rays + r * a.ray_stride, a.ray_stride);
    else { ray.ox = ray.oy = ray.oz = 1e30f; ray.dx = ray.dy = ray.dz = 0.f; ray.tmin = 0.f; ray.last = 0.f; }
    int lo = N, hi = -1;
    if (have) ray_interval<false>(F, ray, N, lo, hi);
    const int wlo = wave_min_i(lo), whi = wave_max_i(hi);

    float T = 1.f, acc = 0.f, dep = 0.f;
    int first = -1, last = -1;
    unsigned napp = 0;
    int nev = 0;
    int ovf_from = 0;

    long long frow[4];
    if constexpr (DENSE) {
#pragma unroll
        for (int j = 0; j < 4; ++j) {
            const int rho = (lane >> 2) + 16 * j;
            const int fx = tx * 8 + (rho & 7), fy = ty * 8 + (rho >> 3);
            frow[j] = (fx < a.img_w && fy < a.img_h) ? ((long long)fy * a.img_w + fx) * N : -1;
        }
    }
    constexpr int kSteps = 2;
    const int i_begin = DENSE ? (wlo & ~15) : wlo, i_end = DENSE ? min(N - 1, whi | 15) : whi;
    const float eps = DENSE ? 0.f : F.term_eps;
    bool dead = false;
#ifdef MT_PROF
    unsigned long long p_coord = 0, p_axes = 0, p_build = 0, p_read = 0, p_act = 0, p_pairs = 0;
    const unsigned long long p_start = __builtin_readcyclecounter();
    unsigned long long p_t = p_start;
#endif
    for (int i = i_begin; i <= i_end; i += kSteps) {
        if (eps > 0.f && (((i - i_begin) & 15) == 0)) {
            dead = T < eps;
// ... 136 lines not shown
            }
        }
#ifdef MT_PROF
        MT_T(p_act); ++p_pairs;
#endif
    }
#ifdef MT_PROF
    if (lane == 0 && a.prof) {
        unsigned long long* o = a.prof + (size_t)(blockIdx.x * 4 + wid) * 8;
        o[0] = p_coord; o[1] = p_axes; o[2] = p_build; o[3] = p_read; o[4] = p_act; o[5] = p_pairs; o[6] = __builtin_readcyclecounter() - p_start;
    }
#endif
    const int Lw = last >= first && first >= 0 ? last - first + 1 : 0;
    if (have) {
        a.acc[r] = acc;
        a.depth[r] = dep + (1.f - acc) * ray.last;
    }
    const bool over = have && napp > (unsigned)a.cap;
    const unsigned n = (have && !over) ? napp : 0u;
    unsigned incl = n;
#pragma unroll
    for (int o = 1; o < 64; o <<= 1) {
        const unsigned t = __shfl_up(incl, o);
        if (lane >= o) incl += t;
    }
    const unsigned total = __shfl(incl, 63);
    const unsigned list = blockIdx.x & 7u;
    unsigned base = 0;
    if (lane == 0 && total) base = atomicAdd(&a.counters[list * kCounterStride], total);
    base = __shfl(base, 0);
    const bool fits = base + total <= a.list_cap;
    if (!fits && total) void_entries(a.app_pos, a.app_ray, list, a.list_cap, base, base + total, lane);
    const unsigned slot0 = list * a.list_cap + base + (incl - n);
    if (have) {
        if (over || !fits) {
            const unsigned k = atomicAdd(a.ovf_count, 1u);
            a.ovf_list[k] = (int)r;
            a.ray_app[r] = make_int4(ovf_from, (int)napp, nev, Lw > 0 ? (first | (Lw << 11)) : 0);
        } else {
            a.ray_app[r] = make_int4((int)slot0, fits ? (int)n : 0, nev, Lw > 0 ? (first | (Lw << 11)) : 0);
            if (fits) {
                const float4* __restrict__ src = a.scratch + (size_t)r * a.cap;
                for (unsigned k = 0; k < n; k += 4) {
                    const float4 e0 = src[k], e1 = src[k + 1 < n ? k + 1 : n - 1], e2 = src[k + 2 < n ? k + 2 : n - 1],
                                 e3 = src[k + 3 < n ? k + 3 : n - 1];
                    a.app_pos[slot0 + k] = e0; a.app_ray[slot0 + k] = (int)r;
                    if (k + 1 < n) { a.app_pos[slot0 + k + 1] = e1; a.app_ray[slot0 + k + 1] = (int)r; }
                    if (k + 2 < n) { a.app_pos[slot0 + k + 2] = e2; a.app_ray[slot0 + k + 2] = (int)r; }
                    if (k + 3 < n) { a.app_pos[slot0 + k + 3] = e3; a.app_ray[slot0 + k + 3] = (int)r; }
                }
            }
        }
    }
}

struct CompactArgs {
    FieldDev F;
    const float* rays; long long n_rays; int ray_stride; int n_samples;
    const float* wbuf;
    int4* ray_app; float4* app_pos; int* app_ray; unsigned* counters; unsigned list_cap;
    unsigned long long* stats;
    const float4* scratch; int cap;
    int finisher;
};
__device__ __forceinline__ void reserve_slots(const CompactArgs& a, long long r, unsigned list, int lane, const int4 ra, unsigned& slot0,
                                              unsigned& napp, int* ovf_slot) {
    slot0 = 0;
    if (lane == 0) {
        bool fits = napp == 0;
        for (unsigned att = 0; att < (unsigned)kLists && !fits; ++att) {
            const unsigned l = (list + att) & (unsigned)(kLists - 1);
            if (a.counters[l * kCounterStride] + napp > a.list_cap) continue;
            const unsigned s0 = atomicAdd(&a.counters[l * kCounterStride], napp);
            if (s0 + napp <= a.list_cap) { slot0 = l * a.list_cap + s0; fits = true; }
            else
                for (unsigned e = s0; e < a.list_cap; ++e) {
                    a.app_pos[(size_t)l * a.list_cap + e] = make_float4(0.f, 0.f, 0.f, 0.f);
                    a.app_ray[(size_t)l * a.list_cap + e] = 0;
                }
        }
        if (fits || !a.finisher) a.ray_app[r] = make_int4((int)slot0, fits ? (int)napp : 0, ra.z, ra.w);
        else {
            a.ray_app[r] = make_int4(-ra.x - 1, (int)napp, ra.z, ra.w);
            *ovf_slot = (int)((unsigned)r | 0x80000000u);
            atomicAdd(&a.counters[kFailEntriesWord], napp);
        }
        if (!fits && !a.finisher && a.stats) a.stats[T2N_STAT_OVERFLOW] = 1ull;
        if (!fits) a.counters[kOverflowWord] = 1u;
        if (!fits) napp = 0;
    }
    slot0 = __shfl(slot0, 0);
    napp = __shfl(napp, 0);
}
__device__ __forceinline__ void compact_span(const CompactArgs& a, long long r, const Ray& ray, int from, int end, unsigned slot0, unsigned run,
                                             int lane) {
    const FieldDev& F = a.F;
    const int N = a.n_samples;
    for (int base = from; base < end; base += 64) {
        const int i = base + lane;
        const float w = i < end ? a.wbuf[r * N + i] : 0.f;
        const bool m = (i < end) & (w > F.thres);
        const unsigned long long bal = __ballot(m);
        if (m) {
            const unsigned pre = (unsigned)__popcll(bal & ((1ull << lane) - 1ull));
            const float z = sample_z<false>(F, ray, i, 0.f);
            float xn, yn, zn;
            sample_point<false>(F, ray, z, xn, yn, zn);
            const unsigned s = slot0 + run + pre;
            a.app_pos[s] = make_float4(xn, yn, zn, w);
            a.app_ray[s] = (int)r;
        }
        run += (unsigned)__popcll(bal);
    }
}
__device__ __forceinline__ void compact_ray_staged(const CompactArgs& a, long long r, unsigned list, int lane, int* ovf_slot) {
    const int4 ra = a.ray_app[r];
    const int first = ra.w & 2047, Lw = ra.w >> 11, from = ra.x;
    unsigned napp = (unsigned)ra.y, slot0;
    reserve_slots(a, r, list, lane, ra, slot0, napp, ovf_slot);
    const unsigned staged = napp < (unsigned)a.cap ? napp : (unsigned)a.cap;
    for (unsigned k = (unsigned)lane; k < staged; k += 64u) {
        a.app_pos[slot0 + k] = a.scratch[(size_t)r * a.cap + k];
        a.app_ray[slot0 + k] = (int)r;
    }
    if (napp > staged) {
        const Ray ray = load_ray(a.F, a.rays + r * a.ray_stride, a.ray_stride);
        compact_span(a, r, ray, from, first + Lw, slot0, staged, lane);
    }
}
__global__ __launch_bounds__(256) void k_compact_list(const CompactArgs a, const unsigned* ovf_count, int* ovf_list) {
    const int lane = threadIdx.x & 63;
    const unsigned n = *ovf_count;
    for (unsigned k = blockIdx.x * 4u + (threadIdx.x >> 6); k < n; k += gridDim.x * 4u)
        compact_ray_staged(a, ovf_list[k], blockIdx.x & 7u, lane, ovf_list + k);
}

__global__ __launch_bounds__(256) void k_dense_fill(const FieldDev F, const float* __restrict__ rays, long long n_rays, int ray_stride, int N,
                                                    float* __restrict__ w, float* __restrict__ z) {
    const int lane = threadIdx.x & 63;
    const long long r = (long long)blockIdx.x * 4 + (threadIdx.x >> 6);
    if (r >= n_rays) return;
    Ray ray;
    if (z) ray = load_ray(F, rays + r * ray_stride, ray_stride);
    for (int i = lane; i < N; i += 64) {
        if (z) z[r * N + i] = sample_z<false>(F, ray, i, 0.f);
        if (w) w[r * N + i] = 0.f;
    }
}

struct SumTableArgs { FactorSet den; float* out; int n[3]; int nb[3]; int shift[3]; long long boxes; };
__global__ __launch_bounds__(256) void k_density_sum_table(const SumTableArgs a) {
    __shared__ __attribute__((aligned(16))) float smem[4 * kStageFloats];
    const int lane = threadIdx.x & 63, wid = threadIdx.x >> 6;
    const long long box = (long long)blockIdx.x * 4 + wid;
    if (box >= a.boxes) return;
    float* __restrict__ stD = smem + (size_t)wid * kStageFloats;
    const int bx = (int)(box % a.nb[0]), by = (int)((box / a.nb[0]) % a.nb[1]), bz = (int)(box / ((long long)a.nb[0] * a.nb[1]));
    const int o[3] = {4 * bx - a.shift[0], 4 * by - a.shift[1], 4 * bz - a.shift[2]};
    const int amn[3] = {max(o[0], 0), max(o[1], 0), max(o[2], 0)};
    table_build<2>(a.den, amn, stD, lane & 15, lane >> 4);
    lds_fence_w();
    table_sum<2>(stD, lane);
    lds_fence_w();
    const int x = amn[0] + (lane & 3), y = amn[1] + ((lane >> 2) & 3), z = amn[2] + (lane >> 4);
    if (x < o[0] + 4 && y < o[1] + 4 && z < o[2] + 4 && x <= a.n[0] && y <= a.n[1] && z <= a.n[2])
        a.out[((size_t)z * (a.n[1] + 1) + y) * (a.n[0] + 1) + x] = stD[lane];
}

size_t density_cache_bytes(const t2n_field* f) {
    const int* g = f->desc.grid;
    return (size_t)(g[0] + 1) * (g[1] + 1) * (g[2] + 1) * sizeof(float);
}

int launch_density_sum_table(const t2n_field* f, float* out, const int shift[3], hipStream_t s) {
    SumTableArgs a;
    a.den = f->dev.den; a.out = out;
    a.boxes = 1;
    for (int k = 0; k < 3; ++k) {
        if (shift[k] < 0 || shift[k] > 3) { set_error("density sum table: shift[%d]=%d outside [0, 3]", k, shift[k]); return T2N_ERR_INVALID; }
        a.n[k] = f->desc.grid[k]; a.shift[k] = shift[k];
        a.nb[k] = (a.n[k] + shift[k]) / 4 + 1;
// ... 16 lines not shown
    f->dcache_seen = f->den_version;
    if (!f->dcache_on) return T2N_OK;
    const int* g = f->desc.grid;
    const size_t bytes = density_cache_bytes(f);
    size_t cap = f->dcache_cap;
    if (!cap) {
        static size_t dev_total = 0;
        if (!dev_total) { size_t fr = 0, tot = 0; if (hipMemGetInfo(&fr, &tot) == hipSuccess) dev_total = tot; else (void)hipGetLastError(); }
        cap = dev_total / 64;
    }
    const bool addressable = (size_t)(g[1] + 1) * (g[2] + 1) < (1u << 24) && bytes < (1ull << 32);
    if ((size_t)g[0] * g[1] * g[2] * sizeof(float) > cap || !addressable) return T2N_OK;
    if (f->dcache && f->dcache_version == f->den_version) {
        if (f->dcache_stream != (void*)s) T2N_HIP(hipStreamWaitEvent(s, (hipEvent_t)f->dcache_ev, 0));
    } else {
        if (!second) return T2N_OK;
        if (!f->dcache) {
            if (f->dcache_alloc_failed) return T2N_OK;
            if (hipMalloc((void**)&f->dcache, bytes + 16) != hipSuccess) {
                (void)hipGetLastError();
                f->dcache = nullptr; f->dcache_alloc_failed = true;
                return T2N_OK;
            }
            f->dcache_bytes = bytes + 16;
        }
        if (!f->dcache_ev) T2N_HIP(hipEventCreateWithFlags((hipEvent_t*)&f->dcache_ev, hipEventDisableTiming));
        const int shift[3] = {0, 0, 0};
        const int rc = launch_density_sum_table(f, f->dcache, shift, s);
        if (rc) return rc;
        T2N_HIP(hipEventRecord((hipEvent_t)f->dcache_ev, s));
        f->dcache_stream = (void*)s;
        f->dcache_version = f->den_version;
        ++f->dcache_counts[2];
    }
    f->dev.dsum = f->dcache;
    f->dev.ds_row = (unsigned)(g[0] + 1) * 4u;
    f->dev.ds_slice = f->dev.ds_row * (unsigned)(g[1] + 1);
    return T2N_OK;
}

int launch_march_tiles(t2n_field* f, const RenderLaunch& L, int img_w, int img_h, float* spill, float4* scratch, hipStream_t s) {
    const int cap = L.n_samples / 4 > 0 ? L.n_samples / 4 : 1;
    unsigned* ovf_count = (unsigned*)((char*)scratch + (size_t)L.n_rays * cap * 16);
    int* ovf_list = (int*)((char*)ovf_count + 256);
    const bool dense = L.weights != nullptr;
    TileArgs a;
    a.F = f->dev;
    a.rays = L.rays; a.n_rays = L.n_rays; a.ray_stride = L.ray_stride; a.n_samples = L.n_samples; a.img_w = img_w; a.img_h = img_h;
    a.acc = L.acc; a.depth = L.depth; a.ray_app = L.ray_app;
    a.wbuf = L.weights ? L.weights : spill;
    a.scratch = scratch; a.cap = cap; a.ovf_count = ovf_count; a.ovf_list = ovf_list;
    a.app_pos = L.app_pos; a.app_ray = L.app_ray; a.counters = L.counters; a.list_cap = L.list_cap; a.stats = (unsigned long long*)L.stats;
    a.dense_w = L.weights;
    a.F.term_eps = (!L.weights && !L.z_vals && !L.sigma_ctx) ? f->term_eps : 0.f;
#ifdef MT_PROF
    static unsigned long long* prof = nullptr;
    static int prof_calls = 0;
    const long long prof_waves = ((long long)((img_w + 7) / 8) * ((img_h + 7) / 8) + 3) / 4 * 4;
    if (!prof) T2N_HIP(hipMalloc((void**)&prof, (size_t)65536 * 8 * 8));
    T2N_HIP(hipMemsetAsync(prof, 0, (size_t)65536 * 8 * 8, s));
    a.prof = prof_waves <= 65536 ? prof : nullptr;
#endif
    const long long tiles = (long long)((img_w + 7) / 8) * ((img_h + 7) / 8);
    const dim3 grid((unsigned)((tiles + 3) / 4));
    timing_begin(f, T2N_K_MARCH, s);
    if (L.weights || L.z_vals)
        hipLaunchKernelGGL(k_dense_fill, dim3((unsigned)((L.n_rays + 3) / 4)), dim3(256), 0, s, f->dev, L.rays, (long long)L.n_rays, L.ray_stride,
                           L.n_samples, L.weights, L.z_vals);
    const bool cached = f->dev.dsum != nullptr;
    const size_t lds = (size_t)4 * ((cached ? 0 : kStageFloats) + (dense ? kDenseFloats : 0)) * sizeof(float);
    const bool mask = f->dev.alpha != nullptr, relu = f->dev.act == T2N_ACT_RELU;
    ++f->dcache_counts[cached ? 0 : 1];
#define T2N_MT_LAUNCH(D, A, R) do { if (cached) hipLaunchKernelGGL((k_march_tiles<D, A, R, true>), grid, dim3(256), lds, s, a); \
                                    else hipLaunchKernelGGL((k_march_tiles<D, A, R, false>), grid, dim3(256), lds, s, a); } while (0)
    if (dense) { if (mask) { if (relu) T2N_MT_LAUNCH(true, true, true); else T2N_MT_LAUNCH(true, true, false); }
                 else { if (relu) T2N_MT_LAUNCH(true, false, true); else T2N_MT_LAUNCH(true, false, false); } }
    else { if (mask) { if (relu) T2N_MT_LAUNCH(false, true, true); else T2N_MT_LAUNCH(false, true, false); }
           else { if (relu) T2N_MT_LAUNCH(false, false, true); else T2N_MT_LAUNCH(false, false, false); } }
#undef T2N_MT_LAUNCH
    T2N_HIP(hipGetLastError());
#ifdef MT_PROF
    if (a.prof && ++prof_calls == 20) {
        static unsigned long long h[65536 * 8];
        T2N_HIP(hipStreamSynchronize(s));
        T2N_HIP(hipMemcpy(h, prof, sizeof(h), hipMemcpyDeviceToHost));
        double sum[8] = {0, 0, 0, 0, 0, 0, 0, 0};
        long long n = 0;
        for (long long i = 0; i < prof_waves; ++i) if (h[i * 8 + 5]) { ++n; for (int k = 0; k < 8; ++k) sum[k] += (double)h[i * 8 + k]; }
        if (n) fprintf(stderr, "[mt prof] %lld waves, per wave: step pairs %.1f, cycles in the step loop %.0f = coordinates + validity %.0f, axis taps + union bit set %.0f, "
                               "table build (loads -> MFMA -> LDS) %.0f, table reads %.0f, activation + compositing + staging %.0f; per step pair %.0f\n",
                       n, sum[5] / n, (sum[0] + sum[1] + sum[2] + sum[3] + sum[4]) / n, sum[0] / n, sum[1] / n, sum[2] / n, sum[3] / n, sum[4] / n,
                       (sum[0] + sum[1] + sum[2] + sum[3] + sum[4]) / (sum[5] > 0 ? sum[5] : 1));
    }
#endif
    CompactArgs c;
    c.F = f->dev;
    c.rays = L.rays; c.n_rays = L.n_rays; c.ray_stride = L.ray_stride; c.n_samples = L.n_samples;
    c.wbuf = a.wbuf;
    c.ray_app = L.ray_app; c.app_pos = L.app_pos; c.app_ray = L.app_ray; c.counters = L.counters; c.list_cap = L.list_cap;
    c.stats = (unsigned long long*)L.stats;
    c.scratch = scratch; c.cap = cap;
    c.finisher = finish_supported(f) ? 1 : 0;
    hipLaunchKernelGGL(k_compact_list, dim3(64), dim3(256), 0, s, c, (const unsigned*)ovf_count, ovf_list);
    timing_end(f, T2N_K_MARCH, s);
    T2N_HIP(hipGetLastError());
    return launch_ray_stats(L, s);
}

}
```

### text2nerf_amd/csrc/t2n_mlp_ss.hip

```cpp
#include "t2n_device.h"

namespace t2n {
namespace ss {

typedef float f32x4 __attribute__((ext_vector_type(4)));
typedef float f32x16 __attribute__((ext_vector_type(16)));
typedef _Float16 h8 __attribute__((ext_vector_type(8)));
typedef _Float16 h2v __attribute__((ext_vector_type(2)));
typedef __fp16 hh2 __attribute__((ext_vector_type(2)));

constexpr int kC0 = 12, kC1 = 4;
constexpr int kS2 = 8;
constexpr int kStep = 4 * 2 * 64;
constexpr int kChunk = 2 * kStep;
constexpr int kRingSlots = 4;
constexpr int kRing = kRingSlots * kChunk;
constexpr int kW0 = kC0 * kChunk;
constexpr int kW1 = kC1 * kChunk;
constexpr int kW2 = kS2 * 2 * 64;
constexpr int kBias = 288;
constexpr size_t kLds = (size_t)(kRing + kW1 + kW2) * 16 + kBias * 4 + 16 * 4;
constexpr float kRange = 59968.f;

struct Args {
// ... 341 lines not shown
    }
}
template <int T_, bool TRACK>
__device__ __forceinline__ void stage(TileCtx& c) {
    if constexpr (T_ > 0) conv_bias<0, 128>(c.V1, c.LBh);
    {
        ConvFill3<0, 64 * T_, 0, TRACK> f{c.H0h, c.H0l, c.V0, c.inv0, c.neg1, c.amax, c.LBh, nullptr};
        f.all();
    }
    stage_step<T_, 0, TRACK>(c); stage_step<T_, 1, TRACK>(c); stage_step<T_, 2, TRACK>(c); stage_step<T_, 3, TRACK>(c);
    stage_step<T_, 4, TRACK>(c); stage_step<T_, 5, TRACK>(c); stage_step<T_, 6, TRACK>(c); stage_step<T_, 7, TRACK>(c);
    if constexpr (T_ + 1 < kT3) conv_bias<0, 0>(c.V0, c.LBh);
    if constexpr (T_ > 0) {
        L2Ops<64 * (T_ - 1), false> l2{c.A2[1], c.H1h[7], c.H1l[7]};
        l2.template run<3>(); l2.template run<7>(); l2.template run<11>();
        SS_FENCE();
    }
}
template <int St, int BASE, class F>
__device__ __forceinline__ void l2_step(AEl (&A2)[2], const u4v& Hh, const u4v& Hl, F& f, const LdsA& L) {
    mfma_acc<BASE, St == 0, true>(A2[St % 2].h, Hh);
    mfma_acc<BASE + 16, St == 0, false>(A2[St % 2].l, Hh);
    mfma_acc<BASE + 32, St == 0, false>(A2[St % 2].h, Hl);
    fetch2<St + 2>(A2, L);
    f.all();
    SS_FENCE();
}

#define SS3_BAR_ASM(KEEP) do { __builtin_amdgcn_s_waitcnt((KEEP) == 0 ? 0x0070 : 0x0074); asm volatile("s_barrier" ::: "memory"); } while (0)
#ifdef SS3_ABL_NO_BARRIER
#define SS3_BARRIER(KEEP) do {} while (0)
#elif defined(SS3_PROF)
#define SS3_BARRIER(KEEP) do { const unsigned long long tb = __builtin_readcyclecounter(); SS3_BAR_ASM(KEEP); p_bar += __builtin_readcyclecounter() - tb; } while (0)
#else
#define SS3_BARRIER(KEEP) SS3_BAR_ASM(KEEP)
#endif
#ifdef SS3_PROF
#define SS3_T(var) do { const unsigned long long tn = __builtin_readcyclecounter(); var += tn - p_t; p_t = tn; } while (0)
#else
#define SS3_T(var) do {} while (0)
#endif
template <int BASE, class F>
__device__ __forceinline__ void l2_last(AEl (&A2)[2], const u4v& Hh, const u4v& Hl, F (&f)[kT3]) {
    mfma_acc<BASE, false, true>(A2[1].h, Hh);
    mfma_acc<BASE + 16, false, false>(A2[1].l, Hh);
    mfma_acc<BASE + 32, false, false>(A2[1].h, Hl);
#define SS3_E(I) f[0].template run<I>(); f[1].template run<I>(); f[2].template run<I>()
    SS3_E(0); SS3_E(1); SS3_E(2); SS3_E(3); SS3_E(4); SS3_E(5); SS3_E(6); SS3_E(7); SS3_E(8); SS3_E(9); SS3_E(10); SS3_E(11);
#undef SS3_E
    f[0].done(); f[1].done(); f[2].done();
    SS_FENCE();
}

template <bool TRACK>
__global__ __launch_bounds__(256) void k_mlp_ss3(const Args a) {
    extern __shared__ __attribute__((aligned(16))) uint4 lds[];
    if ((__float_as_uint(a.bounds[4]) != 0u) == TRACK) return;
    uint4* __restrict__ RING = lds;
    uint4* __restrict__ W1 = RING + kRing;
    uint4* __restrict__ W2 = W1 + kW1;
    float* __restrict__ LB = reinterpret_cast<float*>(W2 + kW2);
    static_assert(kRing * 16 == 65536 && kW1 * 16 == 65536, "the ring and W1 each fill one 64-KB window");
    unsigned* __restrict__ LT = reinterpret_cast<unsigned*>(LB + kBias);
    const int tid = threadIdx.x, lane = tid & 63, w = __builtin_amdgcn_readfirstlane(tid >> 6);
    const int j = lane & 31, h = lane >> 5;
    unsigned ob0 = (unsigned)lane * 16u, ob1 = (unsigned)lane * 16u + 65536u, ob2 = (unsigned)lane * 16u + 131072u,
             obb = (unsigned)((kW2 + kRing + kW1) * 16) + 16u * (unsigned)h;
    asm volatile("" : "+v"(ob0));
    asm volatile("" : "+v"(ob1));
    asm volatile("" : "+v"(ob2));
    asm volatile("" : "+v"(obb));
    const LdsA L{reinterpret_cast<const u4v*>(reinterpret_cast<const char*>(lds) + ob0), reinterpret_cast<const u4v*>(reinterpret_cast<const char*>(lds) + ob1),
                 reinterpret_cast<const u4v*>(reinterpret_cast<const char*>(lds) + ob2)};
    const float* __restrict__ LBh = reinterpret_cast<const float*>(reinterpret_cast<const char*>(lds) + obb);

    unsigned cnt_l = 0;
    if (lane < a.nlists) {
        cnt_l = a.counters[lane * kCounterStride];
        if (cnt_l > a.list_cap) cnt_l = a.list_cap;
    }
    unsigned incl = (cnt_l + 31u) / 32u;
#pragma unroll
    for (int o = 1; o < 8; o <<= 1) {
        const unsigned t = __shfl_up(incl, o);
        if (lane >= o) incl += t;
    }
    unsigned ntiles = __shfl(incl, a.nlists - 1);
    if (ntiles > a.tile_hi) ntiles = a.tile_hi;
    const unsigned nrounds = (ntiles + 11u) / 12u;
    if (blockIdx.x >= nrounds) return;
    if (tid < 8) { LT[tid] = tid < a.nlists ? incl : 0xffffffffu; LT[8 + tid] = cnt_l; }

    const float inv0 = a.inv_scale[0], inv1 = a.inv_scale[1], inv2 = a.inv_scale[2];
    for (int i = tid; i < kW1; i += 256) W1[i] = a.w1[i];
    for (int i = tid; i < kW2; i += 256) W2[i] = a.w2[i];
    for (int i = tid; i < kBias; i += 256) LB[i] = a.bias[i] * (i < 128 ? inv0 : (i < 256 ? inv1 : inv2));
    const Stream3 S{a.w0, tid};
    S.dma<0>(RING, 0); S.dma<1>(RING, 0); S.dma<2>(RING, 0); S.dma<3>(RING, 0);
    S.dma<0>(RING + kChunk, 1); S.dma<1>(RING + kChunk, 1); S.dma<2>(RING + kChunk, 1); S.dma<3>(RING + kChunk, 1);
    S.dma<0>(RING + 2 * kChunk, 2); S.dma<1>(RING + 2 * kChunk, 2); S.dma<2>(RING + 2 * kChunk, 2); S.dma<3>(RING + 2 * kChunk, 2);
    const float neg1 = a.neg1;
    s2v amax = {0, 0};
    unsigned amax_u = 0u;

    const unsigned last = ntiles * 32u - 1u;
    auto load_feat = [&](unsigned r, int t, float (&f)[14]) {
        unsigned i = ((r * 4u + (unsigned)w) * 3u + (unsigned)t) * 32u + (unsigned)j;
        i = i < last ? i : last;
        const float2* __restrict__ row = reinterpret_cast<const float2*>(a.feat + (size_t)i * 32 + 14 * h);
#pragma unroll
        for (int e = 0; e < 7; ++e) { const float2 v = row[e]; f[2 * e] = v.x; f[2 * e + 1] = v.y; }
    };
    float wnext[kT3] = {0.f, 0.f, 0.f};
    auto finish_feat = [&](EncIn& I, float& wn) {
        const float xs = __shfl_xor(I.f[13], 32);
        I.fh = h ? xs : I.f[13];
        I.extra = h ? I.fh : 0.f;
        wn = xs;
    };
    Enc3 E[kT3];
    u4v Bh[2][kT3], Bl[2][kT3];
#pragma unroll
    for (int t = 0; t < kT3; ++t) {
        E[t].in.hs = h ? 8.f : 1.f;
        load_feat(blockIdx.x, t, E[t].in.f);
    }
#pragma unroll
    for (int t = 0; t < kT3; ++t) {
        finish_feat(E[t].in, wnext[t]);
        EncFill3<0> f{E[t], Bh[0][t], Bl[0][t], neg1};
        fill_all(f);
    }
    __syncthreads();
    AEl A[4], A2[2];
    Conv3 V, V1;

#ifdef SS3_PROF
    unsigned long long p_bar = 0, p_l0 = 0, p_tile[3] = {0, 0, 0}, p_top = 0, p_rounds = 0, p_tail = 0;
    const unsigned long long p_start = __builtin_readcyclecounter();
    unsigned long long p_t = p_start;
#endif
    for (unsigned r = blockIdx.x; r < nrounds; r += gridDim.x) {
        float wgt[kT3];
#pragma unroll
        for (int t = 0; t < kT3; ++t) {
#pragma unroll
            for (int e = 0; e < 14; ++e) amax_u = max(amax_u, __float_as_uint(E[t].in.f[e]) & 0x7fffffffu);
            wgt[t] = wnext[t];
        }
        asm volatile("" : "+v"(amax_u));
        const unsigned rn = r + gridDim.x < nrounds ? r + gridDim.x : r;
        SS3_T(p_top);
        asm volatile("; SS3_MARK layer0");
#define SS3_ENC(S_, P_) {{E[0], Bh[P_][0], Bl[P_][0], neg1}, {E[1], Bh[P_][1], Bl[P_][1], neg1}, {E[2], Bh[P_][2], Bl[P_][2], neg1}}
#define SS3_L0(C)                                                                                                                 \
        {                                                                                                                         \
             \
             \
            SS3_BARRIER(C == 9 ? 0 : 4);                                                                                          \
            if constexpr (C == 0) { fetch<0>(A, L); fetch<1>(A, L); fetch<2>(A, L); fetch<3>(A, L); }                             \
            RingOps3 ring{S, RING + ((C + 3) % kRingSlots) * kChunk, (C + 3) % kC0};                                              \
// ... 204 lines not shown
        const int row = lane & 31, kh = lane >> 5;
#pragma unroll
        for (int e = 0; e < 8; ++e) x[e] = row < 3 ? a.w2[row * 128 + hid_unit(st, kh, e)] * s2 : 0.f;
        a.w2p[g] = make_uint4(pack2(x[0], x[1], part), pack2(x[2], x[3], part), pack2(x[4], x[5], part), pack2(x[6], x[7], part));
        return;
    }
    g -= kW2;
    if (g < kBias) {
        float b = 0.f;
        if (g < 128) b = a.b0[g] * s0;
        else if (g < 256) b = a.b1[g - 128] * s1;
        else if (g - 256 < 3) b = a.b2[g - 256] * s2;
        a.biasp[g] = b;
    }
}

}

int ss_pack(t2n_field* f, hipStream_t s) {
    using namespace ss;
    const size_t nw = (size_t)kW0 + kW1 + kW2;
    if (!f->buf_ss) {
        T2N_HIP(hipMalloc((void**)&f->buf_ss, nw * 16 + (kBias + 16) * 4));
    }
    uint4* base = (uint4*)f->buf_ss;
    PackArgs a;
    const t2n_field_params& p = f->params_ref;
    a.w0 = p.mlp_w0; a.b0 = p.mlp_b0; a.w1 = p.mlp_w1; a.b1 = p.mlp_b1; a.w2 = p.mlp_w2; a.b2 = p.mlp_b2;
    a.w0p = base; a.w1p = base + kW0; a.w2p = base + kW0 + kW1;
    a.biasp = (float*)(base + nw); a.scales = a.biasp + kBias;
    hipLaunchKernelGGL(k_ss_scales, dim3(1), dim3(256), 0, s, a);
    const size_t total = nw + kBias;
    hipLaunchKernelGGL(k_pack_ss, dim3((unsigned)((total + 255) / 256)), dim3(256), 0, s, a);
    T2N_HIP(hipGetLastError());
    if (!f->ss_event) { hipEvent_t e; T2N_HIP(hipEventCreateWithFlags(&e, hipEventDisableTiming)); f->ss_event = (void*)e; }
    T2N_HIP(hipEventRecord((hipEvent_t)f->ss_event, s));
    f->ss_stream = (void*)s;
    f->ss_dirty = false;
    f->ss_variant = -1;
    if (!f->ss_ok_host) {
        if (hipHostMalloc((void**)&f->ss_ok_host, 4, hipHostMallocDefault) != hipSuccess) { f->ss_ok_host = nullptr; (void)hipGetLastError(); }
        hipEvent_t e;
        if (f->ss_ok_host && hipEventCreateWithFlags(&e, hipEventDisableTiming) == hipSuccess) f->ss_ok_event = (void*)e;
    }
    if (f->ss_ok_host && f->ss_ok_event) {
        *f->ss_ok_host = 0xffffffffu;
        if (hipMemcpyAsync(f->ss_ok_host, a.scales + 12, 4, hipMemcpyDeviceToHost, s) != hipSuccess ||
            hipEventRecord((hipEvent_t)f->ss_ok_event, s) != hipSuccess) { (void)hipGetLastError(); f->ss_variant = -2; }
    } else f->ss_variant = -2;
    return T2N_OK;
}

int launch_mlp_ss(t2n_field* f, const float* feat, const unsigned* counters_dev, unsigned list_cap, unsigned tile_hi, float4* app_rgb,
                  unsigned* range_flag, hipStream_t s) {
    using namespace ss;
    if (f->ss_dirty || !f->buf_ss) { const int rc = ss_pack(f, s); if (rc) return rc; }
    else if (f->ss_event && f->ss_stream != (void*)s) T2N_HIP(hipStreamWaitEvent(s, (hipEvent_t)f->ss_event, 0));
    static bool attr_set = false;
    if (!attr_set) {
        T2N_HIP(hipFuncSetAttribute((const void*)k_mlp_ss3<true>, hipFuncAttributeMaxDynamicSharedMemorySize, (int)kLds));
        T2N_HIP(hipFuncSetAttribute((const void*)k_mlp_ss3<false>, hipFuncAttributeMaxDynamicSharedMemorySize, (int)kLds));
        attr_set = true;
    }
    const size_t nw = (size_t)kW0 + kW1 + kW2;
    uint4* base = (uint4*)f->buf_ss;
    Args a;
    a.w0 = base; a.w1 = base + kW0; a.w2 = base + kW0 + kW1;
    a.bias = (const float*)(base + nw); a.inv_scale = a.bias + kBias + 4; a.bounds = a.bias + kBias + 8;
    a.feat = feat; a.counters = counters_dev; a.list_cap = list_cap; a.nlists = kLists; a.tile_hi = tile_hi; a.app_rgb = app_rgb;
    a.range_flag = range_flag; a.neg1 = -1.f;
#ifdef SS3_PROF
    static unsigned long long* prof = nullptr;
    static int prof_calls = 0;
    if (!prof) { T2N_HIP(hipMalloc((void**)&prof, 1024 * 10 * 8)); }
    T2N_HIP(hipMemsetAsync(prof, 0, 1024 * 10 * 8, s));
    a.prof = prof;
#endif
    if (f->ss_variant == -1 && hipEventQuery((hipEvent_t)f->ss_ok_event) == hipSuccess && *f->ss_ok_host != 0xffffffffu)
        f->ss_variant = *f->ss_ok_host ? 0 : 1;
    else if (f->ss_variant == -1) (void)hipGetLastError();
    if (f->ss_variant != 1) hipLaunchKernelGGL(k_mlp_ss3<false>, dim3(256), dim3(256), kLds, s, a);
    if (f->ss_variant != 0) hipLaunchKernelGGL(k_mlp_ss3<true>, dim3(256), dim3(256), kLds, s, a);
#ifdef SS3_PROF
    if (++prof_calls == 20) {
        static unsigned long long h[1024 * 10];
        T2N_HIP(hipStreamSynchronize(s));
        T2N_HIP(hipMemcpy(h, prof, sizeof(h), hipMemcpyDeviceToHost));
        double sum[10] = {0, 0, 0, 0, 0, 0, 0, 0, 0, 0};
        for (int i = 0; i < 1024; ++i) for (int k = 0; k < 10; ++k) sum[k] += (double)h[i * 10 + k];
        fprintf(stderr, "[ss3 prof] per wave: barrier-wait %.0f, layer0 (incl. barriers) %.0f, stage0 %.0f, stage1 %.0f, stage2 %.0f, tail %.0f, top %.0f, rounds %.1f, total %.0f cycles\n",
                sum[0] / 1024, sum[1] / 1024, sum[2] / 1024, sum[3] / 1024, sum[4] / 1024, sum[8] / 1024, sum[5] / 1024, sum[6] / 1024, sum[7] / 1024);
    }
#endif
    T2N_HIP(hipGetLastError());
    return T2N_OK;
}

}
```

### text2nerf_amd/csrc/t2n_shade.hip

```cpp
#include "t2n_device.h"

namespace t2n {

typedef float f32x16 __attribute__((ext_vector_type(16)));

constexpr int kXld = 33;
constexpr int kAppK = 144;
constexpr int kTileFloats = kAppK * kXld;
constexpr int kPE = 6;
constexpr int kL0Pairs = 14;
constexpr int kBasisReal = kAppK / 2;
constexpr int kL0Real = kL0Pairs * (1 + 2 * kPE) + 1;
constexpr int kL1Real = 65, kL2Real = 65;
constexpr int kKS1 = 8, kKS4 = 2;
constexpr int kBasisStages = 9, kL0Stages = 93, kL1Stages = 33, kL2Stages = 9;
constexpr int kPadStages = 2;
constexpr int kBasisSteps = (kBasisStages + kPadStages) * kKS1;
constexpr int kL0Steps = (kL0Stages + kPadStages) * kKS4;
constexpr int kL1Steps = (kL1Stages + kPadStages) * kKS4;
constexpr int kL2Steps = (kL2Stages + kPadStages) * kKS1;
static_assert(kBasisStages * kKS1 >= kBasisReal && kL0Stages * kKS4 >= kL0Real && kL1Stages * kKS4 >= kL1Real && kL2Stages * kKS1 >= kL2Real, "stages");

__host__ __device__ constexpr int unit_of(int v, int h) { return (v & 3) + 8 * (v >> 2) + 4 * h; }

// ... 1701 lines not shown
    if (blocks > cap) blocks = cap;
    if (blocks == 0) blocks = 1;
    return (int)blocks;
}

static dim3 grid_redo(const dim3& g) { return dim3(g.x < 256u ? g.x : 256u); }
constexpr size_t kCoopLds = (size_t)4 * kWaveFloats * sizeof(float);
static bool use_coop(const t2n_field* f) {
    return f->mlp_split && f->desc.shading == T2N_SHADE_MLP_FEA_NOVIEW;
}

static bool use_ws(const t2n_field* f) {
    return use_coop(f);
}

static int feature_stage(t2n_field* f, const ShadeArgs& a, unsigned ws_tiles, float* feat, unsigned* flag, bool half, hipStream_t s) {
    if (f->dev.avol) return launch_app_features_vol(f, a.app_pos, a.counters, a.list_cap, ws_tiles, feat, s);
    ShadeArgs fa = a;
    fa.F.shading = T2N_SHADE_RGB;
    fa.app_rgb = nullptr;
    fa.ctx = ShadeCtx{nullptr, feat, nullptr, nullptr};
    fa.ctx_rows = ws_tiles * 32u; fa.tile_hi = ws_tiles;
    fa.range_flag = flag; fa.split_unsafe = f->split_unsafe;
    fa.feature_staging = f->feature_staging; fa.staging_counts = f->staging_counts; fa.defer_cap = f->feature_defer_cap;
    const size_t lds_p = (size_t)kPairBasisVec * 16 + (size_t)kPairWaves * kPairFloats * sizeof(float);
    static bool attr_p = false;
    if (!attr_p) {
        T2N_HIP(hipFuncSetAttribute((const void*)k_app_features_p<false>, hipFuncAttributeMaxDynamicSharedMemorySize, (int)lds_p));
        T2N_HIP(hipFuncSetAttribute((const void*)k_app_features_p<true>, hipFuncAttributeMaxDynamicSharedMemorySize, (int)lds_p));
        attr_p = true;
    }
    const unsigned long long wg = ((unsigned long long)ws_tiles + kPairWaves - 1) / kPairWaves;
    const unsigned wg_max = f->feature_workgroups > 0 ? (unsigned)f->feature_workgroups : 512u;
    const dim3 grid_p((unsigned)(wg < wg_max ? (wg ? wg : 1u) : wg_max));
    if (half) hipLaunchKernelGGL(k_app_features_p<true>, grid_p, dim3(64 * kPairWaves), lds_p, s, fa);
    else hipLaunchKernelGGL(k_app_features_p<false>, grid_p, dim3(64 * kPairWaves), lds_p, s, fa);
    T2N_HIP(hipGetLastError());
    return T2N_OK;
}

int launch_feature_rows(t2n_field* f, const float4* app_pos, const unsigned* counters_dev, unsigned list_cap, float* feat, unsigned feat_rows,
                        hipStream_t s) {
    ShadeArgs a;
    memset(&a, 0, sizeof(a));
    a.tile_lo = 0; a.tile_hi = 0xffffffffu;
    a.F = f->dev;
    a.app_pos = app_pos; a.counters = counters_dev; a.list_cap = list_cap; a.nlists = kLists;
    const bool half = f->factor_bf16 && f->dev.app.plane_h[0];
    return feature_stage(f, a, feat_rows / 32u, feat, const_cast<unsigned*>(counters_dev) + kRangeFlagWord, half, s);
}

int launch_shade_list(t2n_field* f, const float4* app_pos, const int* app_ray, const float* rays, int ray_stride,
                      const unsigned* counters_dev, unsigned list_cap, float4* app_rgb, const ShadeCtx* ctx, hipStream_t s,
                      bool features_only, unsigned ctx_rows, float* feat, unsigned feat_rows, uint64_t* stats, unsigned tile_lo, unsigned tile_hi) {
    ShadeArgs a;
    memset(&a, 0, sizeof(a));
    if (ctx) a.ctx = *ctx;
    a.ctx_rows = ctx_rows;
    a.tile_lo = tile_lo; a.tile_hi = tile_hi;
    a.F = f->dev;
    if (features_only) a.F.shading = T2N_SHADE_RGB;
    a.app_pos = app_pos; a.app_ray = app_ray; a.rays = rays; a.ray_stride = ray_stride;
    a.counters = counters_dev; a.list_cap = list_cap; a.nlists = kLists; a.app_rgb = app_rgb;
    const size_t lds = (size_t)4 * kTileFloats * sizeof(float);
    static bool attr_set = false;
    if (!attr_set) {
        T2N_HIP(hipFuncSetAttribute((const void*)k_shade<false>, hipFuncAttributeMaxDynamicSharedMemorySize, (int)lds));
        T2N_HIP(hipFuncSetAttribute((const void*)k_shade<true>, hipFuncAttributeMaxDynamicSharedMemorySize, (int)lds));
        T2N_HIP(hipFuncSetAttribute((const void*)k_shade_coop<false>, hipFuncAttributeMaxDynamicSharedMemorySize, (int)kCoopLds));
        T2N_HIP(hipFuncSetAttribute((const void*)k_shade_coop<true>, hipFuncAttributeMaxDynamicSharedMemorySize, (int)kCoopLds));
        attr_set = true;
    }
    const dim3 grid(shade_grid((unsigned long long)list_cap * kLists));
    const bool half = f->factor_bf16 && f->dev.app.plane_h[0];
    const unsigned ws_tiles = feat ? feat_rows / 128u * 4u : 0u;
    if (use_ws(f) && !ctx && !features_only && ws_tiles >= 4u) {
        unsigned* flag = const_cast<unsigned*>(counters_dev) + kRangeFlagWord;
        timing_begin(f, T2N_K_APPFEAT, s);
        { const int rc = feature_stage(f, a, ws_tiles, feat, flag, half, s); if (rc) return rc; }
        timing_end(f, T2N_K_APPFEAT, s);
        timing_begin(f, T2N_K_SHADE, s);
        const int rc = launch_mlp_ss(f, feat, counters_dev, list_cap, ws_tiles, app_rgb, flag, s);
        if (rc) return rc;
        ShadeArgs oa = a;
        oa.tile_lo = ws_tiles; oa.range_flag = flag; oa.split_unsafe = f->split_unsafe;
        const dim3 grid_o(grid.x < 64u ? grid.x : 64u);
        if (half) hipLaunchKernelGGL(k_shade_coop<true>, grid_o, dim3(256), kCoopLds, s, oa);
        else hipLaunchKernelGGL(k_shade_coop<false>, grid_o, dim3(256), kCoopLds, s, oa);
        ShadeArgs ra = a;
        ra.run_if_nonzero = counters_dev + kRangeFlagWord; ra.stats = (unsigned long long*)stats;
        hipLaunchKernelGGL(k_shade<false>, grid_redo(grid), dim3(256), lds, s, ra);
        timing_end(f, T2N_K_SHADE, s);
        T2N_HIP(hipGetLastError());
        return T2N_OK;
    }
    unsigned* flag = const_cast<unsigned*>(counters_dev) + kRangeFlagWord;
    a.range_flag = flag; a.split_unsafe = f->split_unsafe;
    timing_begin(f, T2N_K_SHADE, s);
    if (use_coop(f) && !ctx && half) hipLaunchKernelGGL(k_shade_coop<true>, grid, dim3(256), kCoopLds, s, a);
    else if (use_coop(f) && !ctx) hipLaunchKernelGGL(k_shade_coop<false>, grid, dim3(256), kCoopLds, s, a);
    else if (use_coop(f) && ctx && !half && !features_only) {
        static bool attr_c = false;
        if (!attr_c) { T2N_HIP(hipFuncSetAttribute((const void*)k_shade_coop<false, true>, hipFuncAttributeMaxDynamicSharedMemorySize, (int)kCoopLds)); attr_c = true; }
        hipLaunchKernelGGL((k_shade_coop<false, true>), grid, dim3(256), kCoopLds, s, a);
    }
    else if (f->mlp_split)    hipLaunchKernelGGL(k_shade<true>, grid, dim3(256), lds, s, a);
    else hipLaunchKernelGGL(k_shade<false>, grid, dim3(256), lds, s, a);
    if (f->mlp_split) {
        ShadeArgs ra = a;
        ra.range_flag = nullptr; ra.split_unsafe = nullptr;
        ra.run_if_nonzero = flag; ra.stats = (unsigned long long*)stats;
        hipLaunchKernelGGL(k_shade<false>, grid_redo(grid), dim3(256), lds, s, ra);
    }
    timing_end(f, T2N_K_SHADE, s);
    T2N_HIP(hipGetLastError());
    return T2N_OK;
}

}

using namespace t2n;


extern "C" size_t t2n_shade_workspace_bytes(int64_t n) { (void)n; return 256; }

extern "C" int t2n_shade_at(const t2n_field* fc, const float* xyz_norm, const float* viewdirs, int64_t n, float* app_feat,
                            float* rgb, void* workspace, size_t workspace_bytes, t2n_stream stream) {
    t2n_field* f = const_cast<t2n_field*>(fc);
    if (!f || !xyz_norm || n < 0 || n > 0x7fffffff) { set_error("t2n_shade_at: bad argument"); return T2N_ERR_INVALID; }
    if (!f->uploaded) { set_error("t2n_shade_at: field has no uploaded parameters"); return T2N_ERR_STATE; }
    if (f->desc.shading == T2N_SHADE_SH && rgb && !viewdirs) { set_error("t2n_shade_at: SH head needs viewdirs"); return T2N_ERR_INVALID; }
    if (head_is_generic(f->desc.shading) && rgb) { set_error("t2n_shade_at: the view-dependent MLP heads are evaluated by the render call only (features are available)"); return T2N_ERR_UNSUPPORTED; }
    if (n == 0) return T2N_OK;
    if (f->mlp_split && (!workspace || workspace_bytes < 4)) { set_error("t2n_shade_at: workspace smaller than t2n_shade_workspace_bytes()"); return T2N_ERR_INVALID; }
    ShadeArgs a;
// ... 26 lines not shown
```

### text2nerf_amd/tensorf.py

```python
from __future__ import annotations

import ctypes as C
import math
import os
import weakref
import time
from typing import Optional

import numpy as np
import torch
import torch.nn as nn

from . import _lib
from ._lib import FLAG_ADD_BG, FLAG_COHERENT, FLAG_DEVICE_ROWS, FLAG_KEEP_CTX, FLAG_NDC, FLAG_TRAIN, T2NError

MAT_MODE = [[0, 1], [0, 2], [1, 2]]
VEC_MODE = [2, 1, 0]

_SEED_MIN_RAYS = 8192
_WORKSPACE = {}


def _distortion_weight(w) -> float:
    w = float(w)
# ... 283 lines not shown
        super().__init__()
        self.viewpe, self.pospe = viewpe, pospe
        self._build((3 + 2 * viewpe * 3) + (3 + 2 * pospe * 3) + inChanel, featureC)


class MLPRender(_ViewHead):

    def __init__(self, inChanel, viewpe=6, featureC=128):
        super().__init__()
        self.viewpe = viewpe
        self._build((3 + 2 * viewpe * 3) + inChanel, featureC)


class TensorBase(nn.Module):

    def __init__(self, aabb, gridSize, device, density_n_comp=8, appearance_n_comp=24, app_dim=27,
                 shadingMode="MLP_PE", alphaMask=None, near_far=[2.0, 6.0], density_shift=-10, alphaMask_thres=0.001,
                 distance_scale=25, rayMarch_weight_thres=0.0001, pos_pe=6, view_pe=6, fea_pe=6, featureC=128,
                 step_ratio=2.0, fea2denseAct="softplus"):
        super().__init__()
        if isinstance(density_n_comp, int):
            density_n_comp = [density_n_comp] * 3
        if isinstance(appearance_n_comp, int):
            appearance_n_comp = [appearance_n_comp] * 3
        self.density_n_comp = list(density_n_comp)
        self.app_n_comp = list(appearance_n_comp)
        self.app_dim = app_dim
        self.aabb = torch.as_tensor(aabb, dtype=torch.float32).to(device)
        self.alphaMask = alphaMask
        self.device = device
        self.density_shift = density_shift
        self.alphaMask_thres = alphaMask_thres
        self.distance_scale = distance_scale
        self.rayMarch_weight_thres = rayMarch_weight_thres
        self.fea2denseAct = fea2denseAct
        self.near_far = near_far
        self.step_ratio = step_ratio
        self.matMode, self.vecMode, self.comp_w = MAT_MODE, VEC_MODE, [1, 1, 1]
        self.shadingMode, self.pos_pe, self.view_pe, self.fea_pe, self.featureC = shadingMode, pos_pe, view_pe, fea_pe, featureC
        self.keep_activation_rows = True
        self.defer_factor_grads = False
        self.materialize_weights = True
        self.z_gate = 2.0
        self.frame_width = 0
        self.mlp_exact_fp32 = False
        self.feature_stage_shape = (0, 0)
        self.feature_staging = True
        self.factor_storage = "fp32"
        self.density_cache = True
        self.density_cache_cap_bytes = 0
        self.appearance_volume = True
        self.appearance_volume_min_frames = 0
        self.appearance_volume_cap_bytes = 0
        self.early_termination = 0.0
        self._handle = None
        self._uploaded_key = None
        self._gbuf = None
        self._gbuf_dirty = False
        self._gbuf_stale = False
        self.last_stats = None
        self._dcache_base = [0, 0, 0]
        _FIELDS.add(self)

        if shadingMode not in _lib.SHADE_IDS:
            raise T2NError(f"shadingMode {shadingMode!r} is not implemented by the HIP renderer "
                           f"(supported: {sorted(_lib.SHADE_IDS)})")
        self.update_stepSize(gridSize)
        self.init_svd_volume(gridSize[0], device)
        self.init_render_func(shadingMode, pos_pe, view_pe, fea_pe, featureC, device)
        self._is_general()

    def init_render_func(self, shadingMode, pos_pe, view_pe, fea_pe, featureC, device):
        if shadingMode == "MLP_Fea_noview":
            self.renderModule = MLPRender_Fea_noview(self.app_dim, fea_pe, featureC).to(device)
        elif shadingMode == "MLP_PE":
            raise T2NError("shadingMode 'MLP_PE': the reference's MLPRender_PE sizes its first layer for 3 inputs it never "
                           "concatenates (models/tensorBase.py:115 vs :126-131) and fails with a shape error for every "
                           "pos_pe / view_pe; there is no behaviour to reproduce")
        elif shadingMode == "MLP_Fea":
            self.renderModule = MLPRender_Fea(self.app_dim, view_pe, fea_pe, featureC).to(device)
        elif shadingMode == "MLP":
            self.renderModule = MLPRender(self.app_dim, view_pe, featureC).to(device)
        elif shadingMode == "SH":
            self.renderModule = SHRender
        elif shadingMode == "RGB":
            assert self.app_dim == 3
            self.renderModule = RGBRender
        else:
            raise T2NError(f"Unrecognized shading module {shadingMode!r}")

    def _sample(self, rays_o, rays_d, N, jitter, ndc):
        lib = _lib.load()
        h = self.sync_params()
        dev = self.basis_mat.weight.device if hasattr(self, "basis_mat") else self._all_params()[0].device
        o = rays_o.detach().reshape(-1, 3).contiguous().float().to(dev)
        d = rays_d.detach().reshape(-1, 3).contiguous().float().to(dev)
        n = o.shape[0]
        pts = torch.empty(n, N, 3, device=dev, dtype=torch.float32)
        z = None if ndc else torch.empty(n, N, device=dev, dtype=torch.float32)
        valid = torch.empty(n, N, device=dev, dtype=torch.uint8)
        with torch.cuda.device(dev):
            _lib.check(lib.t2n_sample_ray(h, _lib.ptr(o), _lib.ptr(d), n, int(N), _lib.ptr(jitter), 1 if ndc else 0, _lib.ptr(pts),
                                          _lib.ptr(z), _lib.ptr(valid), _lib.current_stream_ptr(dev)), "t2n_sample_ray")
        return pts, z, valid.bool()

    def sample_ray(self, rays_o, rays_d, is_train=True, N_samples=-1):
# ... 296 lines not shown
        dev = self.basis_mat.weight.device
        pre = self.__dict__.get("_gbuf_preseed")
        if not ahead and pre is not None and getattr(self, "_gbuf_stale", False) and pre[:2] == (tv_d, tv_a) and pre[2] == self._factor_key() \
                and pre[4] == reg:
            self.__dict__["_gbuf_preseed"] = None
            self._gbuf_stale = False
            self._gbuf_dirty = True
            self._gbuf_reduced = False
            return pre[3]
        h = self.sync_params()
        self.factor_grad_buffer(_raw=True)
        cur = torch.cuda.current_stream(dev)
        side = self.__dict__.get("_seed_stream")
        if side is None:
            side = self.__dict__["_seed_stream"] = torch.cuda.Stream(device=dev)
        side.wait_stream(cur)
        with torch.cuda.device(dev):
            if any(reg):
                _lib.check(lib.t2n_field_reg_seed(h, tv_d, tv_a, *reg, side.cuda_stream), "t2n_field_reg_seed")
            else:
                _lib.check(lib.t2n_field_tv_seed(h, tv_d, tv_a, side.cuda_stream), "t2n_field_tv_seed")
        ev = side.record_event()
        self._gbuf_dirty = True
        self._gbuf_reduced = False
        if ahead:
            self._gbuf_stale = True
            self.__dict__["_gbuf_preseed"] = (tv_d, tv_a, self._factor_key(), ev, reg)
        else:
            self._gbuf_stale = False
            self.__dict__["_gbuf_preseed"] = None
        return ev

    def sync_params(self, force=False, frame_width=None):
        lib = _lib.load()
        ps = self._all_params()
        dev = ps[0].device
        if dev.type != "cuda":
            raise T2NError(f"TensorVMSplit parameters live on {dev}; the renderer runs on an MI355X (cuda/HIP) only")
        for p in ps:
            if p.dtype != torch.float32 or not p.is_contiguous():
                raise T2NError("parameters must be contiguous float32")
        if self._handle is None:
            h = C.c_void_p()
            d = self._desc()
            _lib.check(lib.t2n_field_create(C.byref(d), C.byref(h)), "t2n_field_create")
            self._handle = h
            self._precision_set = None
            self._term_set = None
            self._storage_set = None
            self._frame_w_set = None
            self._staging_set = None
            self._dcache_set = (True, 0)
            self._avol_set = (True, 0, 0)
            self._stage_shape_set = (0, 0)
            self._head_rows_set = 32
            self._alpha_key = "unset"
        queued = False
        mask = self.alphaMask
        mkey = None if mask is None else (mask.alpha_volume.data_ptr(), mask.alpha_volume._version, tuple(mask.alpha_volume.shape))
        if getattr(self, "_alpha_key", "unset") != mkey:
            queued = True
            self._wait_readers(dev)
            with torch.cuda.device(dev):
                if mask is None:
                    _lib.check(lib.t2n_field_set_alpha_mask(self._handle, None, 0, 0, 0, None, None, _lib.current_stream_ptr(dev)),
                               "t2n_field_set_alpha_mask")
                else:
                    vol = mask.alpha_volume.reshape(mask.alpha_volume.shape[-3:]).contiguous().float().to(dev)
                    amin = (C.c_float * 3)(*mask.aabb[0].float().cpu().tolist())
                    ainv = (C.c_float * 3)(*mask.invgridSize.float().cpu().tolist())
                    D, H, W = vol.shape
                    _lib.check(lib.t2n_field_set_alpha_mask(self._handle, _lib.ptr(vol), D, H, W, amin, ainv,
                                                            _lib.current_stream_ptr(dev)), "t2n_field_set_alpha_mask")
                    object.__setattr__(mask, "_field", self)
            self._alpha_key = mkey
        hr = int(getattr(self, "head_scratch_rows_per_ray", 32))
        if getattr(self, "_head_rows_set", 32) != hr:
            _lib.check(lib.t2n_field_set_head_scratch_rows(self._handle, hr), "t2n_field_set_head_scratch_rows")
            self._head_rows_set = hr
        fw = int(self.frame_width if frame_width is None else frame_width)
        if getattr(self, "_frame_w_set", None) != fw:
            _lib.check(lib.t2n_field_set_frame_width(self._handle, fw), "t2n_field_set_frame_width")
            self._frame_w_set = fw
        if self._precision_set != bool(self.mlp_exact_fp32):
            _lib.check(lib.t2n_field_set_mlp_precision(self._handle, 1 if self.mlp_exact_fp32 else 0),
                       "t2n_field_set_mlp_precision")
            self._precision_set = bool(self.mlp_exact_fp32)
        if getattr(self, "_staging_set", None) != bool(self.feature_staging):
            _lib.check(lib.t2n_field_set_feature_staging(self._handle, 1 if self.feature_staging else 0),
                       "t2n_field_set_feature_staging")
            self._staging_set = bool(self.feature_staging)
        dc = (bool(getattr(self, "density_cache", True)), int(getattr(self, "density_cache_cap_bytes", 0)))
        if getattr(self, "_dcache_set", (True, 0)) != dc:
            _lib.check(lib.t2n_field_set_density_cache(self._handle, 1 if dc[0] else 0), "t2n_field_set_density_cache")
            _lib.check(lib.t2n_field_set_density_cache_cap(self._handle, dc[1]), "t2n_field_set_density_cache_cap")
            self._dcache_set = dc
        av = (bool(getattr(self, "appearance_volume", True)), int(getattr(self, "appearance_volume_min_frames", 0)),
              int(getattr(self, "appearance_volume_cap_bytes", 0)))
        if getattr(self, "_avol_set", (True, 0, 0)) != av:
            _lib.check(lib.t2n_field_set_appearance_volume(self._handle, 1 if av[0] else 0, av[1]), "t2n_field_set_appearance_volume")
            _lib.check(lib.t2n_field_set_appearance_volume_cap(self._handle, av[2]), "t2n_field_set_appearance_volume_cap")
            self._avol_set = av
        shape = tuple(int(v) for v in self.feature_stage_shape)
        if getattr(self, "_stage_shape_set", (0, 0)) != shape:
            _lib.check(lib.t2n_field_set_feature_stage_shape(self._handle, shape[0], shape[1]), "t2n_field_set_feature_stage_shape")
            self._stage_shape_set = shape
        et = max(0.0, min(float(self.early_termination or 0.0), float(self.rayMarch_weight_thres)))
        if getattr(self, "_term_set", None) != et:
            _lib.check(lib.t2n_field_set_early_termination(self._handle, et), "t2n_field_set_early_termination")
            self._term_set = et
        if self.factor_storage not in ("fp32", "bf16"):
            raise T2NError(f"factor_storage {self.factor_storage!r}: expected 'fp32' or 'bf16'")
        if getattr(self, "_storage_set", None) != self.factor_storage:
            _lib.check(lib.t2n_field_set_factor_storage(self._handle, 1 if self.factor_storage == "bf16" else 0),
                       "t2n_field_set_factor_storage")
            self._storage_set = self.factor_storage
            force = True
        key = tuple((p.data_ptr(), p._version) for p in ps)
        if force or key != self._uploaded_key:
            self._wait_readers(dev)
            with torch.cuda.device(dev):
                st = self._param_struct([p.detach() for p in ps])
                if not force and self._uploaded_key is not None and key[:12] == getattr(self, "_device_factor_key", None):
                    _lib.check(lib.t2n_field_upload_head(self._handle, C.byref(st), _lib.current_stream_ptr(dev)),
                               "t2n_field_upload_head")
                else:
                    _lib.check(lib.t2n_field_upload(self._handle, C.byref(st), _lib.current_stream_ptr(dev)),
                               "t2n_field_upload")
            self._uploaded_key = key
            self._device_factor_key = key[:12]
            queued = True
        cur = torch.cuda.current_stream(dev)
        if queued:
            ev = torch.cuda.Event()
            ev.record(cur)
            self._upload_event, self._upload_seen, self._upload_stream = ev, {int(cur.cuda_stream)}, int(cur.cuda_stream)
        elif getattr(self, "_upload_event", None) is not None and int(cur.cuda_stream) not in self._upload_seen:
            cur.wait_event(self._upload_event)
            self._upload_seen.add(int(cur.cuda_stream))
        return self._handle

    def _wait_readers(self, dev):
        readers = self.__dict__.get("_reader_events")
        if readers:
            cur = torch.cuda.current_stream(dev)
            for sid, ev in readers.items():
                if sid != int(cur.cuda_stream):
                    cur.wait_event(ev)
            readers.clear()

    def _note_reader(self, dev):
        seen = getattr(self, "_upload_seen", None)
        cur = torch.cuda.current_stream(dev)
        sid = int(cur.cuda_stream)
        if seen is None or sid == getattr(self, "_upload_stream", sid):
# ... 669 lines not shown

    def _poll_device_rows(self):
        if not getattr(self, "device_rows_steps", 0) or self._handle is None:
            return True
        rec = (C.c_uint32 * 10)()
        _lib.check(_lib.load().t2n_field_device_rows_record(self._handle, rec), "t2n_field_device_rows_record")
        if rec[9] < getattr(self, "_device_rows_issued", 0):
            self.device_rows_unanswered = getattr(self, "device_rows_unanswered", 0) + 1
        margin = getattr(self, "_device_rows_margin", 1.25)
        seen = getattr(self, "_device_rows_ovf_seen", 0)
        overflowed = rec[8] > seen
        if overflowed:
            self.device_rows_overflows = getattr(self, "device_rows_overflows", 0) + int(rec[8] - seen)
            self._device_rows_ovf_seen = int(rec[8])
            margin = min(2.0, margin * 1.25)
            self._device_rows_clean = 0
        else:
            self._device_rows_clean = getattr(self, "_device_rows_clean", 0) + 1
            if self._device_rows_clean >= 64:
                margin, self._device_rows_clean = max(1.25, margin / 1.1), 0
        self._device_rows_margin = margin
        need = max(rec[0:8])
        if need:
            self._ctx_rows_hint = (int(need * margin) + 95) // 32 * 32
        return not overflowed

    def stats(self):
        s = self.last_stats.cpu().tolist()
        if s[_lib.STAT_OVERFLOW]:
            raise T2NError("appearance list overflow — workspace sizing bug")
        return {"evaluated": s[_lib.STAT_EVALUATED], "appearance": s[_lib.STAT_APPEARANCE], "f16_redo": s[_lib.STAT_F16_REDO],
                "list_retry": s[_lib.STAT_LIST_RETRY]}

    def feature_staging_counts(self):
        if self._handle is None:
            return (0, 0)
        out = (C.c_uint64 * 2)()
        _lib.check(_lib.load().t2n_field_feature_staging_counts(self._handle, out), "t2n_field_feature_staging_counts")
        return (int(out[0]), int(out[1]))

    def density_cache_counts(self):
        base = self.__dict__.get("_dcache_base", [0, 0, 0])
        out = (C.c_uint64 * 4)()
        if self._handle is not None:
            _lib.check(_lib.load().t2n_field_density_cache_counts(self._handle, out), "t2n_field_density_cache_counts")
        return {"cached": base[0] + int(out[0]), "uncached": base[1] + int(out[1]), "builds": base[2] + int(out[2]), "bytes": int(out[3])}

    def appearance_volume_counts(self):
        out = (C.c_uint64 * 4)()
        if self._handle is not None:
            _lib.check(_lib.load().t2n_field_appearance_volume_counts(self._handle, out), "t2n_field_appearance_volume_counts")
        return {"bytes": int(out[0]), "builds": int(out[1]), "volume": int(out[2]), "direct": int(out[3])}

    def density_sum_table(self, shift=(0, 0, 0)):
        h = self.sync_params()
        g = [int(v) for v in self.gridSize]
        dev = self._all_params()[0].device
        out = torch.empty((g[2] + 1, g[1] + 1, g[0] + 1), dtype=torch.float32, device=dev)
        sh = (C.c_int * 3)(*[int(v) for v in shift])
        with torch.cuda.device(dev):
            _lib.check(_lib.load().t2n_field_density_sum_table(h, sh, _lib.ptr(out), _lib.current_stream_ptr(dev)), "t2n_field_density_sum_table")
        return out


class TensorVMSplit(TensorBase):

    def __init__(self, aabb, gridSize, device, **kargs):
        super().__init__(aabb, gridSize, device, **kargs)

    def init_svd_volume(self, res, device):
        self.density_plane, self.density_line = self.init_one_svd(self.density_n_comp, self.gridSize, 0.1, device)
        self.app_plane, self.app_line = self.init_one_svd(self.app_n_comp, self.gridSize, 0.1, device)
        self.basis_mat = nn.Linear(sum(self.app_n_comp), self.app_dim, bias=False).to(device)

    def init_one_svd(self, n_component, gridSize, scale, device):
        planes, lines = [], []
        g = [int(x) for x in gridSize]
        for i in range(3):
            m0, m1 = MAT_MODE[i]
            planes.append(nn.Parameter(scale * torch.randn((1, n_component[i], g[m1], g[m0]))))
            lines.append(nn.Parameter(scale * torch.randn((1, n_component[i], g[VEC_MODE[i]], 1))))
        return nn.ParameterList(planes).to(device), nn.ParameterList(lines).to(device)

    def get_optparam_groups(self, lr_init_spatialxyz=0.02, lr_init_network=0.001):
        groups = [{"params": self.density_line, "lr": lr_init_spatialxyz},
                  {"params": self.density_plane, "lr": lr_init_spatialxyz},
                  {"params": self.app_line, "lr": lr_init_spatialxyz},
                  {"params": self.app_plane, "lr": lr_init_spatialxyz},
                  {"params": self.basis_mat.parameters(), "lr": lr_init_network}]
        if isinstance(self.renderModule, nn.Module):
            groups += [{"params": self.renderModule.parameters(), "lr": lr_init_network}]
        return groups

    def TV_loss_density(self, reg):
        from .losses import tv_planes
        fused = tv_planes(reg, list(self.density_plane), 1e-2)
        if fused is not None:
            return fused
        total = 0
        for p in self.density_plane:
            total = total + reg(p) * 1e-2
        return total

    def TV_loss_app(self, reg):
        from .losses import tv_planes
        fused = tv_planes(reg, list(self.app_plane), 1e-2)
# ... 355 lines not shown
```

Baseline: 180.6 billion ray-samples/s.

## Fuse appearance feature rows into march via slot-addressed list rows

```diff
diff --git a/include/t2n.h b/include/t2n.h
--- a/include/t2n.h
+++ b/include/t2n.h
@@ -113,6 +113,9 @@
 int t2n_field_set_appearance_volume_cap(t2n_field* f, uint64_t bytes);
 int t2n_field_release_appearance_volume(t2n_field* f);
 int t2n_field_appearance_volume_counts(const t2n_field* f, uint64_t out[4]);
+int t2n_field_set_feature_fusion(t2n_field* f, int on);
+int t2n_field_feature_fusion_counts(const t2n_field* f, uint64_t out[2]);
+int t2n_render_list_shape(int64_t n_rays, int n_samples, int entries_per_ray, uint64_t out[6]);
 int t2n_field_feature_rows(t2n_field* f, const float* app_pos, const uint32_t* counters, uint32_t list_cap, int volume, float* feat,
                            uint32_t feat_rows, t2n_stream stream);
 int t2n_field_set_feature_stage_shape(t2n_field* f, int workgroups, int defer_cap);
diff --git a/text2nerf_amd/_lib.py b/text2nerf_amd/_lib.py
--- a/text2nerf_amd/_lib.py
+++ b/text2nerf_amd/_lib.py
@@ -108,6 +108,9 @@
     "t2n_field_set_appearance_volume_cap": (C.c_int, [C.c_void_p, C.c_uint64]),
     "t2n_field_release_appearance_volume": (C.c_int, [C.c_void_p]),
     "t2n_field_appearance_volume_counts": (C.c_int, [C.c_void_p, C.POINTER(C.c_uint64)]),
+    "t2n_field_set_feature_fusion": (C.c_int, [C.c_void_p, C.c_int]),
+    "t2n_field_feature_fusion_counts": (C.c_int, [C.c_void_p, C.POINTER(C.c_uint64)]),
+    "t2n_render_list_shape": (C.c_int, [C.c_int64, C.c_int, C.c_int, C.POINTER(C.c_uint64)]),
     "t2n_field_feature_rows": (C.c_int, [C.c_void_p, C.c_void_p, C.c_void_p, C.c_uint32, C.c_int, C.c_void_p, C.c_uint32, C.c_void_p]),
     "t2n_field_density_sum_table": (C.c_int, [C.c_void_p, C.POINTER(C.c_int), C.c_void_p, C.c_void_p]),
     "t2n_sample_ray": (C.c_int, [C.c_void_p, C.c_void_p, C.c_void_p, C.c_int64, C.c_int, C.c_void_p, C.c_int, C.c_void_p, C.c_void_p,
diff --git a/text2nerf_amd/build.py b/text2nerf_amd/build.py
--- a/text2nerf_amd/build.py
+++ b/text2nerf_amd/build.py
@@ -69,8 +69,8 @@
                                f"registers, {scratch} B of scratch): the hand-allocated accumulators are not safe with this build")
         if verbose:
             print(f"check_ss3_isa: {name} ok ({body.count('v_accvgpr_read_b32')} accumulator reads, no writes, no spills)", flush=True)
-    if found != 2:
-        raise RuntimeError(f"check_ss3_isa: expected the two instantiations of k_mlp_ss3 in the assembly, found {found}")
+    if found != 4:
+        raise RuntimeError(f"check_ss3_isa: expected the four instantiations of k_mlp_ss3 in the assembly, found {found}")
 
 
 def build(force=False, verbose=False):
diff --git a/text2nerf_amd/csrc/t2n_api.hip b/text2nerf_amd/csrc/t2n_api.hip
--- a/text2nerf_amd/csrc/t2n_api.hip
+++ b/text2nerf_amd/csrc/t2n_api.hip
@@ -353,7 +353,8 @@
     c.sigma = o; if (ctx) o = align_up(o + (size_t)rays * n_samples * 4, 256);
     c.rgb_raw = o; if (ctx) o = align_up(o + (size_t)rays * 16, 256);
     c.scratch = o; if (ctx) o = align_up(o + (size_t)rays * (size_t)(n_samples / 4 > 0 ? n_samples / 4 : 1) * 16 + 256 + (size_t)rays * 4, 256);
-    const size_t worst_rows = cap + (size_t)kLists * 32, want_rows = (size_t)rays * (budget && budget < 64 ? (budget + 1) / 2 : 32) + 1024;
+    const bool budgeted = budget && budget < 64 && budget < (unsigned)n_samples;
+    const size_t worst_rows = cap + (size_t)kLists * 32, want_rows = budgeted ? cap : (size_t)rays * 32 + 1024;
     c.feat_rows = (unsigned)(((worst_rows < want_rows ? worst_rows : want_rows) + 127) / 128 * 128);
     if (!feat) c.feat_rows = 0;
     c.feat = o; o = align_up(o + (size_t)c.feat_rows * 32 * sizeof(float), 256);
@@ -727,6 +728,7 @@
         L.app_pos = (float4*)(ws + c.app_pos); L.app_rgb = (float4*)(ws + c.app_rgb); L.app_ray = (int*)(ws + c.app_ray);
         L.list_cap = c.list_cap;
         L.feat = (float*)(ws + c.feat); L.feat_rows = c.feat_rows;
+        L.slot_rows = tiles && f->fusion_on && f->dev.dsum && f->dev.avol && !f->dev.alpha && !weights && !keep && !generic_head && fuse_rows(c.list_cap, c.feat_rows);
         L.sigma_ctx = keep ? (float*)(ws + c.sigma) : nullptr;
         L.rgb_raw = keep ? (float4*)(ws + c.rgb_raw) : nullptr;
         int rc;
@@ -784,7 +786,7 @@
                 ShadeCtx ctx{(float*)(ws + kr.x144), (float*)(ws + kr.feat32), (float*)(ws + kr.h0), (float*)(ws + kr.h1)};
                 if ((rc = launch_shade_list(f, L.app_pos, L.app_ray, L.rays, ray_stride, L.counters, L.list_cap, L.app_rgb, &ctx, s, false, kr.rows))) return rc;
             } else if ((rc = launch_shade_list(f, L.app_pos, L.app_ray, L.rays, ray_stride, L.counters, L.list_cap, L.app_rgb, nullptr, s, false,
-                                               0xffffffffu, keep ? nullptr : L.feat, L.feat_rows, stats))) return rc;
+                                               0xffffffffu, keep ? nullptr : L.feat, L.feat_rows, stats, 0, 0xffffffffu, L.slot_rows))) return rc;
         }
         if ((rc = tiles ? launch_composite(f, L, s, f->frame_w, (int)(cnt / f->frame_w)) : launch_composite(f, L, s))) return rc;
         if (tiles && finish_supported(f) && (rc = launch_finish_rays(f, L, (const float*)(ws + c.sigma), (const float4*)(ws + c.scratch), s))) return rc;
@@ -797,7 +799,7 @@
     counts_poll(const_cast<t2n_field*>(f), false);
     const size_t worst = carve(n_rays, n_samples).total;
     if (n_rays < kBudgetMinRays) return worst;
-    unsigned b = f->list_hint ? 2u * f->list_hint + 16u : 32u;
+    unsigned b = f->list_hint ? f->list_hint + f->list_hint / 2u + 12u : 32u;
     if (b < kBudgetMin) b = kBudgetMin;
     if (b >= (unsigned)n_samples) return worst;
     const size_t want = carve_workspace(n_rays, n_samples, true, true, b).total;
@@ -913,6 +915,23 @@
 extern "C" int t2n_field_appearance_volume_counts(const t2n_field* f, uint64_t out[4]) {
     if (!f || !out) { set_error("t2n_field_appearance_volume_counts: NULL argument"); return T2N_ERR_INVALID; }
     out[0] = (uint64_t)f->avol_bytes; out[1] = f->avol_counts[2]; out[2] = f->avol_counts[0]; out[3] = f->avol_counts[1];
+    return T2N_OK;
+}
+extern "C" int t2n_field_set_feature_fusion(t2n_field* f, int on) {
+    if (!f) { set_error("t2n_field_set_feature_fusion: NULL field"); return T2N_ERR_INVALID; }
+    f->fusion_on = on ? 1 : 0;
+    return T2N_OK;
+}
+extern "C" int t2n_field_feature_fusion_counts(const t2n_field* f, uint64_t out[2]) {
+    if (!f || !out) { set_error("t2n_field_feature_fusion_counts: NULL argument"); return T2N_ERR_INVALID; }
+    out[0] = f->fusion_counts[0]; out[1] = f->fusion_counts[1];
+    return T2N_OK;
+}
+extern "C" int t2n_render_list_shape(int64_t n_rays, int n_samples, int entries_per_ray, uint64_t out[6]) {
+    if (n_rays <= 0 || n_samples <= 0 || entries_per_ray < 0 || !out) { set_error("t2n_render_list_shape: bad argument"); return T2N_ERR_INVALID; }
+    const Carve c = carve_workspace(n_rays, n_samples, true, true, (unsigned)entries_per_ray);
+    out[0] = c.list_cap; out[1] = c.feat_rows; out[2] = fuse_rows(c.list_cap, c.feat_rows) ? 1 : 0;
+    out[3] = c.app_pos; out[4] = c.feat; out[5] = c.counters;
     return T2N_OK;
 }
 extern "C" int t2n_field_feature_rows(t2n_field* f, const float* app_pos, const uint32_t* counters, uint32_t list_cap, int volume, float* feat,
diff --git a/text2nerf_amd/csrc/t2n_app_rows.h b/text2nerf_amd/csrc/t2n_app_rows.h
--- /dev/null
+++ b/text2nerf_amd/csrc/t2n_app_rows.h
@@ -0,0 +1,71 @@
+#pragma once
+#include "t2n_internal.h"
+#include "t2n_device.h"
+
+namespace t2n {
+
+struct AvVolume { const float* avol; unsigned row, slice, ny1; };
+
+template <int LPE>
+__device__ __forceinline__ void av_feature_row(const FactorSet& app, const AvVolume& v, const float4 mine, const bool live, const int q,
+                                               float* __restrict__ row, const bool store) {
+    constexpr int NQ = 8 / LPE;
+    const char* __restrict__ V = reinterpret_cast<const char*>(v.avol);
+    const Axes3 A = sample_axes_inbox(app, mine.x, mine.y, mine.z);
+    const unsigned ix = (unsigned)min(max(A.a[0].i0, 0), app.W[0] - 1), iy = (unsigned)min(max(A.a[1].i0, 0), app.H[0] - 1);
+    const unsigned iz = (unsigned)min(max(A.a[2].i0, 0), app.H[1] - 1);
+    const unsigned cell = umad24(umad24(iz, v.ny1, iy), v.row, ix * kAvCornerBytes);
+    const unsigned o00 = (live ? cell : 0u) + (unsigned)q * 16u;
+    const unsigned o01 = o00 + v.row, o10 = o00 + v.slice, o11 = o10 + v.row;
+    const unsigned off[4] = {o00, o01, o10, o11};
+    float4 c[4][2][NQ];
+#pragma unroll
+    for (int zy = 0; zy < 4; ++zy)
+#pragma unroll
+        for (int x = 0; x < 2; ++x)
+#pragma unroll
+            for (int i = 0; i < NQ; ++i)
+                c[zy][x][i] = *reinterpret_cast<const float4*>(V + (size_t)off[zy] + ((int)kAvCornerBytes * x + 16 * LPE * i));
+    __builtin_amdgcn_sched_barrier(0);
+    const float wx0 = live ? A.a[0].w0 : 0.f, wx1 = live ? A.a[0].w1 : 0.f;
+    const float wyx[2][2] = {{A.a[1].w0 * wx0, A.a[1].w0 * wx1}, {A.a[1].w1 * wx0, A.a[1].w1 * wx1}};
+    const float wz[2] = {A.a[2].w0, A.a[2].w1};
+    float4 r[NQ];
+#pragma unroll
+    for (int zy = 0; zy < 4; ++zy)
+#pragma unroll
+        for (int x = 0; x < 2; ++x) {
+            const float w = wyx[zy & 1][x] * wz[zy >> 1];
+#pragma unroll
+            for (int i = 0; i < NQ; ++i) r[i] = (zy == 0 && x == 0) ? f4_mul(c[0][0][i], w) : f4_fma(c[zy][x][i], w, r[i]);
+        }
+    if (q == 6 % LPE) r[6 / LPE].w = live ? mine.w : 0.f;
+    if (q == 7 % LPE) r[7 / LPE] = make_float4(0.f, 0.f, 0.f, 0.f);
+    if (store) {
+#pragma unroll
+        for (int i = 0; i < NQ; ++i) *reinterpret_cast<float4*>(row + 4 * LPE * i) = r[i];
+    }
+}
+
+__device__ __forceinline__ void av_slot_rows(const FactorSet& app, const AvVolume& v, const float4* pos, float* feat, unsigned count, int lane) {
+    typedef unsigned u32x4_t __attribute__((ext_vector_type(4)));
+    const int e = lane >> 3, q = lane & 7;
+    const auto rsrc = __builtin_amdgcn_make_buffer_rsrc(const_cast<float4*>(pos), 0, (int)(count * 16u), 0x00020000);
+#pragma unroll 1
+    for (unsigned c0 = 0; c0 < count; c0 += 64u) {
+        const unsigned left = count - c0;
+        const unsigned mine_i = (unsigned)lane < left ? c0 + (unsigned)lane : count - 1u;
+        const u32x4_t p = __builtin_amdgcn_raw_buffer_load_b128(rsrc, (int)(mine_i * 16u), 0, 16);
+        const unsigned npass = left < 64u ? (left + 7u) >> 3 : 8u;
+#pragma unroll 1
+        for (unsigned s = 0; s < npass; ++s) {
+            const int src = (int)(8u * s) + e;
+            const float4 mine = make_float4(__uint_as_float(__shfl(p.x, src)), __uint_as_float(__shfl(p.y, src)),
+                                            __uint_as_float(__shfl(p.z, src)), __uint_as_float(__shfl(p.w, src)));
+            const bool live = (unsigned)src < left;
+            av_feature_row<8>(app, v, mine, live, q, feat + (size_t)(c0 + (unsigned)src) * 32u + 4u * (unsigned)q, live);
+        }
+    }
+}
+
+}
diff --git a/text2nerf_amd/csrc/t2n_app_volume.hip b/text2nerf_amd/csrc/t2n_app_volume.hip
--- a/text2nerf_amd/csrc/t2n_app_volume.hip
+++ b/text2nerf_amd/csrc/t2n_app_volume.hip
@@ -1,5 +1,6 @@
 #include "t2n_internal.h"
 #include "t2n_device.h"
+#include "t2n_app_rows.h"
 
 namespace t2n {
 
@@ -56,7 +57,7 @@
 };
 
 __global__ __launch_bounds__(256) void k_app_features_vol(const AvReadArgs a) {
-    constexpr int LPE = 4, NQ = 8 / LPE, EPP = 64 / LPE, PASSES = 32 / EPP;
+    constexpr int LPE = 4, EPP = 64 / LPE, PASSES = 32 / EPP;
     const int lane = threadIdx.x & 63, wid = __builtin_amdgcn_readfirstlane((int)(threadIdx.x >> 6));
     unsigned cnt_l = 0;
     if (lane < a.nlists) {
@@ -73,7 +74,7 @@
     if (ntiles > a.tile_hi) ntiles = a.tile_hi;
     const unsigned wave_stride = gridDim.x * 4u;
     const int e = lane / LPE, q = lane % LPE;
-    const char* __restrict__ V = reinterpret_cast<const char*>(a.avol);
+    const AvVolume vol{a.avol, a.row, a.slice, a.ny1};
     for (unsigned tile = blockIdx.x * 4u + wid; tile < ntiles; tile += wave_stride) {
         const int li = (int)__popcll(__ballot((lane < a.nlists) & (incl <= tile)));
         const unsigned before = li ? __shfl(incl, li - 1) : 0u;
@@ -92,39 +93,7 @@
         for (int p = 0; p < PASSES; ++p) {
             const bool live = (unsigned)(EPP * p + e) < nlive;
             const float4 mine = pos[p];
-            const Axes3 A = sample_axes_inbox(a.app, mine.x, mine.y, mine.z);
-            const unsigned ix = (unsigned)min(max(A.a[0].i0, 0), a.app.W[0] - 1), iy = (unsigned)min(max(A.a[1].i0, 0), a.app.H[0] - 1);
-            const unsigned iz = (unsigned)min(max(A.a[2].i0, 0), a.app.H[1] - 1);
-            const unsigned cell = umad24(umad24(iz, a.ny1, iy), a.row, ix * kAvCornerBytes);
-            const unsigned o00 = (live ? cell : 0u) + (unsigned)q * 16u;
-            const unsigned o01 = o00 + a.row, o10 = o00 + a.slice, o11 = o10 + a.row;
-            const unsigned off[4] = {o00, o01, o10, o11};
-            float4 c[4][2][NQ];
-#pragma unroll
-            for (int zy = 0; zy < 4; ++zy)
-#pragma unroll
-                for (int x = 0; x < 2; ++x)
-#pragma unroll
-                    for (int i = 0; i < NQ; ++i)
-                        c[zy][x][i] = *reinterpret_cast<const float4*>(V + (size_t)off[zy] + ((int)kAvCornerBytes * x + 16 * LPE * i));
-            __builtin_amdgcn_sched_barrier(0);
-            const float wx0 = live ? A.a[0].w0 : 0.f, wx1 = live ? A.a[0].w1 : 0.f;
-            const float wyx[2][2] = {{A.a[1].w0 * wx0, A.a[1].w0 * wx1}, {A.a[1].w1 * wx0, A.a[1].w1 * wx1}};
-            const float wz[2] = {A.a[2].w0, A.a[2].w1};
-            float4 r[NQ];
-#pragma unroll
-            for (int zy = 0; zy < 4; ++zy)
-#pragma unroll
-                for (int x = 0; x < 2; ++x) {
-                    const float w = wyx[zy & 1][x] * wz[zy >> 1];
-#pragma unroll
-                    for (int i = 0; i < NQ; ++i) r[i] = (zy == 0 && x == 0) ? f4_mul(c[0][0][i], w) : f4_fma(c[zy][x][i], w, r[i]);
-                }
-            if (q == 6 % LPE) r[6 / LPE].w = live ? mine.w : 0.f;
-            if (q == 7 % LPE) r[7 / LPE] = make_float4(0.f, 0.f, 0.f, 0.f);
-            float* __restrict__ row = rb + (unsigned)((EPP * p + e) * 32 + 4 * q);
-#pragma unroll
-            for (int i = 0; i < NQ; ++i) *reinterpret_cast<float4*>(row + 4 * LPE * i) = r[i];
+            av_feature_row<LPE>(a.app, vol, mine, live, q, rb + (unsigned)((EPP * p + e) * 32 + 4 * q), true);
         }
     }
 }
diff --git a/text2nerf_amd/csrc/t2n_internal.h b/text2nerf_amd/csrc/t2n_internal.h
--- a/text2nerf_amd/csrc/t2n_internal.h
+++ b/text2nerf_amd/csrc/t2n_internal.h
@@ -133,6 +133,8 @@
     bool avol_alloc_failed = false;
     void* avol_ev = nullptr; void* avol_stream = nullptr;
     unsigned long long avol_counts[3] = {0, 0, 0};
+    int fusion_on = 1;
+    unsigned long long fusion_counts[2] = {0, 0};
 };
 
 namespace t2n {
@@ -158,6 +160,7 @@
     const float* jitter; float* rgb; float* depth; float* weights; float* z_vals; uint64_t* stats;
     float* acc; int4* ray_app; unsigned* counters; float4* app_pos; int* app_ray; float4* app_rgb; unsigned list_cap;
     float* feat = nullptr; unsigned feat_rows = 0;
+    bool slot_rows = false;
     float* sigma_ctx; float4* rgb_raw;
 };
 int launch_march(t2n_field* f, const RenderLaunch& L, hipStream_t s);
@@ -186,6 +189,7 @@
                         hipStream_t s);
 int launch_march_tiles(t2n_field* f, const RenderLaunch& L, int img_w, int img_h, float* spill, float4* scratch, hipStream_t s);
 constexpr int kLists = 8;
+inline bool fuse_rows(unsigned list_cap, unsigned feat_rows) { return feat_rows && (unsigned long long)list_cap * kLists <= feat_rows; }
 constexpr int kCounterStride = 64;
 inline unsigned list_capacity(long long n_rays, int n_samples) {
     const unsigned nblocks = (unsigned)((n_rays + 3) / 4);
@@ -201,7 +205,7 @@
 int launch_shade_list(t2n_field* f, const float4* app_pos, const int* app_ray, const float* rays, int ray_stride,
                       const unsigned* counters_dev, unsigned list_cap, float4* app_rgb, const ShadeCtx* ctx, hipStream_t s,
                       bool features_only = false, unsigned ctx_rows = 0xffffffffu, float* feat = nullptr, unsigned feat_rows = 0,
-                      uint64_t* stats = nullptr, unsigned tile_lo = 0, unsigned tile_hi = 0xffffffffu);
+                      uint64_t* stats = nullptr, unsigned tile_lo = 0, unsigned tile_hi = 0xffffffffu, bool slot_rows = false);
 constexpr int kRangeFlagWord = 32;
 constexpr int kKeptMagicWord = 33, kKeptRowsWord = 34;
 constexpr int kOverflowWord = 35;
@@ -209,7 +213,7 @@
 constexpr int kFailEntriesWord = 36;
 constexpr unsigned kKeptMagic = 0x4b455054u;
 int launch_mlp_ss(t2n_field* f, const float* feat, const unsigned* counters_dev, unsigned list_cap, unsigned tile_hi, float4* app_rgb,
-                  unsigned* range_flag, hipStream_t s);
+                  unsigned* range_flag, hipStream_t s, bool slot_rows = false);
 
 struct HeadDims { int shading, C, fea_pe, view_pe, pos_pe, o_feat, o_view, o_pe_a, n_pe_a, o_pe_v, n_pe_v, K0, K0pad; };
 HeadDims head_dims(const t2n_field_desc& d);
diff --git a/text2nerf_amd/csrc/t2n_march_tiles.hip b/text2nerf_amd/csrc/t2n_march_tiles.hip
--- a/text2nerf_amd/csrc/t2n_march_tiles.hip
+++ b/text2nerf_amd/csrc/t2n_march_tiles.hip
@@ -1,4 +1,5 @@
 #include "t2n_device.h"
+#include "t2n_app_rows.h"
 
 namespace t2n {
 
@@ -18,6 +19,7 @@
     float4* scratch; int cap; unsigned* ovf_count; int* ovf_list;
     float4* app_pos; int* app_ray; unsigned* counters; unsigned list_cap; unsigned long long* stats;
     float* dense_w;
+    float* feat;
 #ifdef MT_PROF
     unsigned long long* prof;
 #endif
@@ -179,6 +181,14 @@
     }
 }
 
+__device__ __forceinline__ void slot_rows(const FieldDev& F, const float4* __restrict__ app_pos, float* __restrict__ feat, size_t slot,
+                                          unsigned count, int lane) {
+    if (!count) return;
+    asm volatile("s_waitcnt vmcnt(0)" ::: "memory");
+    const AvVolume vol{F.avol, F.av_row, F.av_slice, (unsigned)F.app.H[0] + 1u};
+    av_slot_rows(F.app, vol, app_pos + slot, feat + slot * 32u, count, lane);
+}
+
 constexpr int kDenseLd = 20;
 constexpr int kDenseFloats = 64 * kDenseLd;
 struct __attribute__((aligned(4))) F4U { float x, y, z, w; };
@@ -201,7 +211,7 @@
 #define MT_T(var) do {} while (0)
 #endif
 constexpr int mt_waves(bool dense, bool cached) { return cached ? (dense ? T2N_MTCD_WAVES : T2N_MTC_WAVES) : (dense ? T2N_MTD_WAVES : T2N_MT_WAVES); }
-template <bool DENSE, bool ALPHA = false, bool RELU = false, bool CACHED = false>
+template <bool DENSE, bool ALPHA = false, bool RELU = false, bool CACHED = false, bool ROWS = false>
 __global__ __launch_bounds__(256) __attribute__((amdgpu_waves_per_eu(mt_waves(DENSE, CACHED), mt_waves(DENSE, CACHED)))) void k_march_tiles(const TileArgs a) {
     extern __shared__ __attribute__((aligned(16))) float smem[];
     const int lane = threadIdx.x & 63, wid = threadIdx.x >> 6;
@@ -444,6 +454,15 @@
             }
         }
     }
+    if constexpr (ROWS) {
+        static_assert(CACHED && !DENSE, "rows in the tail: cached, weight-free frames only");
+#ifndef T2N_MT_NO_TAIL_ROWS
+        const unsigned ubase = (unsigned)__builtin_amdgcn_readfirstlane((int)base), utotal = (unsigned)__builtin_amdgcn_readfirstlane((int)total);
+        unsigned cnt = utotal;
+        if (ubase + utotal > a.list_cap) cnt = ubase < a.list_cap ? a.list_cap - ubase : 0u;
+        slot_rows(F, a.app_pos, a.feat, (size_t)list * a.list_cap + ubase, cnt, lane);
+#endif
+    }
 }
 
 struct CompactArgs {
@@ -454,23 +473,26 @@
     unsigned long long* stats;
     const float4* scratch; int cap;
     int finisher;
+    float* feat;
 };
 __device__ __forceinline__ void reserve_slots(const CompactArgs& a, long long r, unsigned list, int lane, const int4 ra, unsigned& slot0,
                                               unsigned& napp, int* ovf_slot) {
     slot0 = 0;
+    napp = (unsigned)__builtin_amdgcn_readfirstlane((int)napp);
+    bool fits = napp == 0;
+    for (unsigned att = 0; att < (unsigned)kLists && !fits; ++att) {
+        const unsigned l = (list + att) & (unsigned)(kLists - 1);
+        unsigned s0 = 0xffffffffu;
+        if (lane == 0 && a.counters[l * kCounterStride] + napp <= a.list_cap) s0 = atomicAdd(&a.counters[l * kCounterStride], napp);
+        s0 = (unsigned)__builtin_amdgcn_readfirstlane((int)s0);
+        if (s0 == 0xffffffffu) continue;
+        if (s0 + napp <= a.list_cap) { slot0 = l * a.list_cap + s0; fits = true; }
+        else if (s0 < a.list_cap) {
+            void_entries(a.app_pos, a.app_ray, l, a.list_cap, s0, a.list_cap, lane);
+            if (a.feat) slot_rows(a.F, a.app_pos, a.feat, (size_t)l * a.list_cap + s0, a.list_cap - s0, lane);
+        }
+    }
     if (lane == 0) {
-        bool fits = napp == 0;
-        for (unsigned att = 0; att < (unsigned)kLists && !fits; ++att) {
-            const unsigned l = (list + att) & (unsigned)(kLists - 1);
-            if (a.counters[l * kCounterStride] + napp > a.list_cap) continue;
-            const unsigned s0 = atomicAdd(&a.counters[l * kCounterStride], napp);
-            if (s0 + napp <= a.list_cap) { slot0 = l * a.list_cap + s0; fits = true; }
-            else
-                for (unsigned e = s0; e < a.list_cap; ++e) {
-                    a.app_pos[(size_t)l * a.list_cap + e] = make_float4(0.f, 0.f, 0.f, 0.f);
-                    a.app_ray[(size_t)l * a.list_cap + e] = 0;
-                }
-        }
         if (fits || !a.finisher) a.ray_app[r] = make_int4((int)slot0, fits ? (int)napp : 0, ra.z, ra.w);
         else {
             a.ray_app[r] = make_int4(-ra.x - 1, (int)napp, ra.z, ra.w);
@@ -479,10 +501,8 @@
         }
         if (!fits && !a.finisher && a.stats) a.stats[T2N_STAT_OVERFLOW] = 1ull;
         if (!fits) a.counters[kOverflowWord] = 1u;
-        if (!fits) napp = 0;
-    }
-    slot0 = __shfl(slot0, 0);
-    napp = __shfl(napp, 0);
+    }
+    if (!fits) napp = 0;
 }
 __device__ __forceinline__ void compact_span(const CompactArgs& a, long long r, const Ray& ray, int from, int end, unsigned slot0, unsigned run,
                                              int lane) {
@@ -519,6 +539,7 @@
         const Ray ray = load_ray(a.F, a.rays + r * a.ray_stride, a.ray_stride);
         compact_span(a, r, ray, from, first + Lw, slot0, staged, lane);
     }
+    if (a.feat) slot_rows(a.F, a.app_pos, a.feat, (size_t)slot0, napp, lane);
 }
 __global__ __launch_bounds__(256) void k_compact_list(const CompactArgs a, const unsigned* ovf_count, int* ovf_list) {
     const int lane = threadIdx.x & 63;
@@ -641,6 +662,10 @@
     a.scratch = scratch; a.cap = cap; a.ovf_count = ovf_count; a.ovf_list = ovf_list;
     a.app_pos = L.app_pos; a.app_ray = L.app_ray; a.counters = L.counters; a.list_cap = L.list_cap; a.stats = (unsigned long long*)L.stats;
     a.dense_w = L.weights;
+    const bool rows = L.slot_rows && f->dev.dsum != nullptr && f->dev.avol != nullptr && !dense && !f->dev.alpha;
+    if (L.slot_rows && !rows) { set_error("launch_march_tiles: a fused frame needs the cached table, the feature volume, no mask and no weights rows"); return T2N_ERR_STATE; }
+    a.feat = rows ? L.feat : nullptr;
+    ++f->fusion_counts[rows ? 0 : 1];
     a.F.term_eps = (!L.weights && !L.z_vals && !L.sigma_ctx) ? f->term_eps : 0.f;
 #ifdef MT_PROF
     static unsigned long long* prof = nullptr;
@@ -660,7 +685,8 @@
     const size_t lds = (size_t)4 * ((cached ? 0 : kStageFloats) + (dense ? kDenseFloats : 0)) * sizeof(float);
     const bool mask = f->dev.alpha != nullptr, relu = f->dev.act == T2N_ACT_RELU;
     ++f->dcache_counts[cached ? 0 : 1];
-#define T2N_MT_LAUNCH(D, A, R) do { if (cached) hipLaunchKernelGGL((k_march_tiles<D, A, R, true>), grid, dim3(256), lds, s, a); \
+#define T2N_MT_LAUNCH(D, A, R) do { if (rows) hipLaunchKernelGGL((k_march_tiles<D, A, R, true, !D && !A>), grid, dim3(256), lds, s, a); \
+                                    else if (cached) hipLaunchKernelGGL((k_march_tiles<D, A, R, true>), grid, dim3(256), lds, s, a); \
                                     else hipLaunchKernelGGL((k_march_tiles<D, A, R, false>), grid, dim3(256), lds, s, a); } while (0)
     if (dense) { if (mask) { if (relu) T2N_MT_LAUNCH(true, true, true); else T2N_MT_LAUNCH(true, true, false); }
                  else { if (relu) T2N_MT_LAUNCH(true, false, true); else T2N_MT_LAUNCH(true, false, false); } }
@@ -690,6 +716,7 @@
     c.stats = (unsigned long long*)L.stats;
     c.scratch = scratch; c.cap = cap;
     c.finisher = finish_supported(f) ? 1 : 0;
+    c.feat = a.feat;
     hipLaunchKernelGGL(k_compact_list, dim3(64), dim3(256), 0, s, c, (const unsigned*)ovf_count, ovf_list);
     timing_end(f, T2N_K_MARCH, s);
     T2N_HIP(hipGetLastError());
diff --git a/text2nerf_amd/csrc/t2n_mlp_ss.hip b/text2nerf_amd/csrc/t2n_mlp_ss.hip
--- a/text2nerf_amd/csrc/t2n_mlp_ss.hip
+++ b/text2nerf_amd/csrc/t2n_mlp_ss.hip
@@ -417,7 +417,7 @@
     SS_FENCE();
 }
 
-template <bool TRACK>
+template <bool TRACK, bool SLOT = false>
 __global__ __launch_bounds__(256) void k_mlp_ss3(const Args a) {
     extern __shared__ __attribute__((aligned(16))) uint4 lds[];
     if ((__float_as_uint(a.bounds[4]) != 0u) == TRACK) return;
@@ -455,6 +455,8 @@
     const unsigned nrounds = (ntiles + 11u) / 12u;
     if (blockIdx.x >= nrounds) return;
     if (tid < 8) { LT[tid] = tid < a.nlists ? incl : 0xffffffffu; LT[8 + tid] = cnt_l; }
+    const unsigned incl_m = lane < a.nlists ? incl : 0xffffffffu;
+    const unsigned s_ntiles = SLOT ? (unsigned)__builtin_amdgcn_readfirstlane((int)ntiles) : 0u;
 
     const float inv0 = a.inv_scale[0], inv1 = a.inv_scale[1], inv2 = a.inv_scale[2];
     for (int i = tid; i < kW1; i += 256) W1[i] = a.w1[i];
@@ -470,8 +472,20 @@
 
     const unsigned last = ntiles * 32u - 1u;
     auto load_feat = [&](unsigned r, int t, float (&f)[14]) {
-        unsigned i = ((r * 4u + (unsigned)w) * 3u + (unsigned)t) * 32u + (unsigned)j;
-        i = i < last ? i : last;
+        unsigned i;
+        if constexpr (SLOT) {
+            unsigned tile = (unsigned)__builtin_amdgcn_readfirstlane((int)((r * 4u + (unsigned)w) * 3u + (unsigned)t));
+            tile = tile < s_ntiles ? tile : s_ntiles - 1u;
+            const int li = (int)__popcll(__ballot(incl_m <= tile));
+            const unsigned before = li ? (unsigned)__builtin_amdgcn_readlane((int)incl_m, li - 1) : 0u;
+            const unsigned cnt = (unsigned)__builtin_amdgcn_readlane((int)cnt_l, li);
+            const unsigned lbase = (unsigned)li * a.list_cap, lastl = lbase + cnt - 1u;
+            i = lbase + (tile - before) * 32u + (unsigned)j;
+            i = i < lastl ? i : lastl;
+        } else {
+            i = ((r * 4u + (unsigned)w) * 3u + (unsigned)t) * 32u + (unsigned)j;
+            i = i < last ? i : last;
+        }
         const float2* __restrict__ row = reinterpret_cast<const float2*>(a.feat + (size_t)i * 32 + 14 * h);
 #pragma unroll
         for (int e = 0; e < 7; ++e) { const float2 v = row[e]; f[2 * e] = v.x; f[2 * e + 1] = v.y; }
@@ -782,7 +796,7 @@
 }
 
 int launch_mlp_ss(t2n_field* f, const float* feat, const unsigned* counters_dev, unsigned list_cap, unsigned tile_hi, float4* app_rgb,
-                  unsigned* range_flag, hipStream_t s) {
+                  unsigned* range_flag, hipStream_t s, bool slot_rows) {
     using namespace ss;
     if (f->ss_dirty || !f->buf_ss) { const int rc = ss_pack(f, s); if (rc) return rc; }
     else if (f->ss_event && f->ss_stream != (void*)s) T2N_HIP(hipStreamWaitEvent(s, (hipEvent_t)f->ss_event, 0));
@@ -790,6 +804,8 @@
     if (!attr_set) {
         T2N_HIP(hipFuncSetAttribute((const void*)k_mlp_ss3<true>, hipFuncAttributeMaxDynamicSharedMemorySize, (int)kLds));
         T2N_HIP(hipFuncSetAttribute((const void*)k_mlp_ss3<false>, hipFuncAttributeMaxDynamicSharedMemorySize, (int)kLds));
+        T2N_HIP(hipFuncSetAttribute((const void*)(k_mlp_ss3<true, true>), hipFuncAttributeMaxDynamicSharedMemorySize, (int)kLds));
+        T2N_HIP(hipFuncSetAttribute((const void*)(k_mlp_ss3<false, true>), hipFuncAttributeMaxDynamicSharedMemorySize, (int)kLds));
         attr_set = true;
     }
     const size_t nw = (size_t)kW0 + kW1 + kW2;
@@ -809,8 +825,13 @@
     if (f->ss_variant == -1 && hipEventQuery((hipEvent_t)f->ss_ok_event) == hipSuccess && *f->ss_ok_host != 0xffffffffu)
         f->ss_variant = *f->ss_ok_host ? 0 : 1;
     else if (f->ss_variant == -1) (void)hipGetLastError();
-    if (f->ss_variant != 1) hipLaunchKernelGGL(k_mlp_ss3<false>, dim3(256), dim3(256), kLds, s, a);
-    if (f->ss_variant != 0) hipLaunchKernelGGL(k_mlp_ss3<true>, dim3(256), dim3(256), kLds, s, a);
+    if (slot_rows) {
+        if (f->ss_variant != 1) hipLaunchKernelGGL((k_mlp_ss3<false, true>), dim3(256), dim3(256), kLds, s, a);
+        if (f->ss_variant != 0) hipLaunchKernelGGL((k_mlp_ss3<true, true>), dim3(256), dim3(256), kLds, s, a);
+    } else {
+        if (f->ss_variant != 1) hipLaunchKernelGGL(k_mlp_ss3<false>, dim3(256), dim3(256), kLds, s, a);
+        if (f->ss_variant != 0) hipLaunchKernelGGL(k_mlp_ss3<true>, dim3(256), dim3(256), kLds, s, a);
+    }
 #ifdef SS3_PROF
     if (++prof_calls == 20) {
         static unsigned long long h[1024 * 10];
diff --git a/text2nerf_amd/csrc/t2n_shade.hip b/text2nerf_amd/csrc/t2n_shade.hip
--- a/text2nerf_amd/csrc/t2n_shade.hip
+++ b/text2nerf_amd/csrc/t2n_shade.hip
@@ -1777,7 +1777,8 @@
 
 int launch_shade_list(t2n_field* f, const float4* app_pos, const int* app_ray, const float* rays, int ray_stride,
                       const unsigned* counters_dev, unsigned list_cap, float4* app_rgb, const ShadeCtx* ctx, hipStream_t s,
-                      bool features_only, unsigned ctx_rows, float* feat, unsigned feat_rows, uint64_t* stats, unsigned tile_lo, unsigned tile_hi) {
+                      bool features_only, unsigned ctx_rows, float* feat, unsigned feat_rows, uint64_t* stats, unsigned tile_lo, unsigned tile_hi,
+                      bool slot_rows) {
     ShadeArgs a;
     memset(&a, 0, sizeof(a));
     if (ctx) a.ctx = *ctx;
@@ -1798,14 +1799,18 @@
     }
     const dim3 grid(shade_grid((unsigned long long)list_cap * kLists));
     const bool half = f->factor_bf16 && f->dev.app.plane_h[0];
-    const unsigned ws_tiles = feat ? feat_rows / 128u * 4u : 0u;
+    const unsigned ws_tiles = slot_rows ? (unsigned)kLists * ((list_cap + 31u) / 32u) : (feat ? feat_rows / 128u * 4u : 0u);
+    if (slot_rows && !(use_ws(f) && !ctx && !features_only && feat && fuse_rows(list_cap, feat_rows))) {
+        set_error("launch_shade_list: slot-addressed rows need the fused MLP_Fea_noview head and a row per list slot");
+        return T2N_ERR_STATE;
+    }
     if (use_ws(f) && !ctx && !features_only && ws_tiles >= 4u) {
         unsigned* flag = const_cast<unsigned*>(counters_dev) + kRangeFlagWord;
         timing_begin(f, T2N_K_APPFEAT, s);
-        { const int rc = feature_stage(f, a, ws_tiles, feat, flag, half, s); if (rc) return rc; }
+        if (!slot_rows) { const int rc = feature_stage(f, a, ws_tiles, feat, flag, half, s); if (rc) return rc; }
         timing_end(f, T2N_K_APPFEAT, s);
         timing_begin(f, T2N_K_SHADE, s);
-        const int rc = launch_mlp_ss(f, feat, counters_dev, list_cap, ws_tiles, app_rgb, flag, s);
+        const int rc = launch_mlp_ss(f, feat, counters_dev, list_cap, ws_tiles, app_rgb, flag, s, slot_rows);
         if (rc) return rc;
         ShadeArgs oa = a;
         oa.tile_lo = ws_tiles; oa.range_flag = flag; oa.split_unsafe = f->split_unsafe;
diff --git a/text2nerf_amd/tensorf.py b/text2nerf_amd/tensorf.py
--- a/text2nerf_amd/tensorf.py
+++ b/text2nerf_amd/tensorf.py
@@ -359,6 +359,7 @@
         self.appearance_volume = True
         self.appearance_volume_min_frames = 0
         self.appearance_volume_cap_bytes = 0
+        self.feature_fusion = True
         self.early_termination = 0.0
         self._handle = None
         self._uploaded_key = None
@@ -761,6 +762,7 @@
             self._staging_set = None
             self._dcache_set = (True, 0)
             self._avol_set = (True, 0, 0)
+            self._fusion_set = True
             self._stage_shape_set = (0, 0)
             self._head_rows_set = 32
             self._alpha_key = "unset"
@@ -810,6 +812,10 @@
             _lib.check(lib.t2n_field_set_appearance_volume(self._handle, 1 if av[0] else 0, av[1]), "t2n_field_set_appearance_volume")
             _lib.check(lib.t2n_field_set_appearance_volume_cap(self._handle, av[2]), "t2n_field_set_appearance_volume_cap")
             self._avol_set = av
+        fu = bool(getattr(self, "feature_fusion", True))
+        if getattr(self, "_fusion_set", True) != fu:
+            _lib.check(lib.t2n_field_set_feature_fusion(self._handle, 1 if fu else 0), "t2n_field_set_feature_fusion")
+            self._fusion_set = fu
         shape = tuple(int(v) for v in self.feature_stage_shape)
         if getattr(self, "_stage_shape_set", (0, 0)) != shape:
             _lib.check(lib.t2n_field_set_feature_stage_shape(self._handle, shape[0], shape[1]), "t2n_field_set_feature_stage_shape")
@@ -1585,6 +1591,12 @@
             _lib.check(_lib.load().t2n_field_appearance_volume_counts(self._handle, out), "t2n_field_appearance_volume_counts")
         return {"bytes": int(out[0]), "builds": int(out[1]), "volume": int(out[2]), "direct": int(out[3])}
 
+    def feature_fusion_counts(self):
+        out = (C.c_uint64 * 2)()
+        if self._handle is not None:
+            _lib.check(_lib.load().t2n_field_feature_fusion_counts(self._handle, out), "t2n_field_feature_fusion_counts")
+        return {"fused": int(out[0]), "unfused": int(out[1])}
+
     def density_sum_table(self, shift=(0, 0, 0)):
         h = self.sync_params()
         g = [int(v) for v in self.gridSize]
```

Measured after the change: 192.1 billion ray-samples/s (median of 6 runs). +6.4%, better.
